# joeyee/Onet

Measured on AMD Instinct MI355X. Metric: training images/sec (twin 256x256 pass), higher is better.
Workload: dtype f32

## Files before the change

### include/onet_hip.h

```cpp
#ifndef ONET_HIP_H
#define ONET_HIP_H

#include <stdint.h>

#ifdef __cplusplus
extern "C" {
#endif

#define ONET_OK 0
#define ONET_EINVAL (-1)
#define ONET_EHIP (-2)

const char* onet_last_error(void);
int onet_abi_version(void);
int onet_device_info(int* cu_count, int* lds_bytes, int* wave_size, char* arch, int arch_len);

int onet_conv3x3_pack_weights(const float* w, float* wp_fwd, float* wp_dgrad,
                              int Cout, int Cin, void* stream);
int onet_convT2x2_pack_weights(const float* w, float* wp_fwd, float* wp_dgrad,
                               int Cin, int Cout, void* stream);
int onet_convT2x2_pack_weights_fused(const float* w, float* wq, int Cin, int Cout, void* stream);
int onet_convT2x2_fwd(const float* x, int64_t x_bs, const float* wq, const float* bias, float* y, int64_t y_bs,
                      int B, int Cin, int Ct, int h, int w, int Ho, int Wo, int pt, int pl, int operand_bf16,
        void* stream);
// ... 4 lines not shown
int onet_convT2x2_dgrad_dbias(const float* dy, int64_t dy_bs, const float* wp_dgrad, float* dx, int64_t dx_bs, float* dbias,
                              void* ws, int64_t ws_bytes, int B, int Cin, int Ct, int h, int w, int Ho, int Wo, int pt, int pl, int operand_bf16,
        void* stream);
int64_t onet_convT2x2_wgrad_ws_bytes(int B, int Cin, int Ct, int h, int w);
int onet_convT2x2_wgrad(const float* x, int64_t x_bs, const float* dy, int64_t dy_bs, float* dw, void* ws,
                        int64_t ws_bytes, int B, int Cin, int Ct, int h, int w, int Ho, int Wo, int pt, int pl, int operand_bf16,
        void* stream);
int onet_convT2x2_dbias(const float* dy, int64_t dy_bs, float* dbias, double* scratch, int accumulate, int B,
                        int C, int h, int w, int Ho, int Wo, int pt, int pl, void* stream);

int onet_conv_fwd(const float* x, int64_t x_bs, const float* wp, float* z, int64_t z_bs,
                  float* bn_part, int B, int Cin, int Cout, int H, int W, int ks, void* stream);
int onet_conv_fwd_nparts(int B, int Cout, int H, int W);

int onet_conv3x3_pack_weights_winograd4(const float* w, float* wq_fwd, float* wq_dgrad,
                                        int Cout, int Cin, void* stream);
int onet_conv3x3_winograd4_fwd(const float* x, int64_t x_bs, const float* wq, float* z, int64_t z_bs,
                               int B, int Cin, int Cout, int H, int W, void* stream);
int onet_conv3x3_winograd4_nparts(int B, int H, int W);
int onet_conv3x3_winograd4_fwd_stats(const float* x, int64_t x_bs, const float* wq, float* z, int64_t z_bs,
                                     float* part, int B, int Cin, int Cout, int H, int W, void* stream);
int onet_conv3x3_winograd4_dgrad_bnreduce(const float* dz, int64_t dz_bs, const float* wq_dgrad, float* da,
                                          int64_t da_bs, const float* z_prev, int64_t z_prev_bs,
                                          const float* save_prev, int group_images, float* part2,
                                          int B, int Cdz, int Cda, int H, int W, void* stream);
int onet_convT2x2_fwd_p(const float* x, int64_t x_bs, const float* wq, const float* bias, void* yP, int64_t yP_bs, const void* y_amax,
                        int nparts, int B, int Cin, int Ct, int h, int w, int Ho, int Wo, int pt, int pl, int operand_bf16, void* stream);
int onet_convT2x2_pack_weights_slots(const float* w, void* wP, void* wdP, void* amax_ws, int Cin, int Ct, int nparts, void* stream);
int onet_convT2x2_fwd_slots(const void* xP, int64_t xP_bs, const void* x_amax, const void* wP, const float* bias, void* yP, int64_t yP_bs,
                            const void* y_amax, int nparts, int B, int Cin, int Ct, int h, int w, void* stream);
int onet_convT2x2_dgrad_slots(const void* dyP, int64_t dyP_bs, const void* dy_amax, const void* wdP, float* dx, int64_t dx_bs, int nparts, int B,
                              int Cin, int Ct, int h, int w, void* stream);
int64_t onet_convT2x2_wgrad_slots_ws_bytes(int B, int Cin, int Ct, int h, int w);
int onet_convT2x2_wgrad_slots(const void* xP, int64_t xP_bs, const void* x_amax, const void* dyP, int64_t dyP_bs, const void* dy_amax, float* dw,
                              float* dbias, void* ws, int64_t ws_bytes, int nparts, int B, int Cin, int Ct, int h, int w, void* stream);
int onet_convT2x2_out_bound(const float* w, const float* bias, int Cin, int Ct, const void* x_amax, void* y_amax, void* stream);

int onet_conv3x3_split_pack_weights(const float* w, void* wq_fwd, void* wq_dgrad, void* amax_ws, int Cout, int Cin, int fwd_f16,
                                    int dgrad_f16, void* stream);
int onet_absmax_slots(const float* x, int64_t n, void* slots, void* stream);
int onet_conv3x3_split_conv_amax(const float* x, int64_t x_bs, const void* x_amax, int scale_always, const void* wq, float* z, int64_t z_bs,
                                 float* part, int B, int Cin, int Cout, int H, int W, void* stream);
int onet_conv3x3_split_wgrad_f16(const float* x, int64_t x_bs, const void* x_amax, const float* save, int n_groups, const float* dz,
                                 int64_t dz_bs, const void* dz_amax, float* dw, void* ws, int64_t ws_bytes, int B, int Cin, int Cout,
                                 int H, int W, int accumulate, void* stream);
int onet_conv3x3_split_fwd(const float* x, int64_t x_bs, const void* wq, int wq_f16, float* z, int64_t z_bs, int B, int Cin, int Cout,
                           int H, int W, void* stream);
int onet_conv3x3_split_nparts(int B, int H, int W);
int onet_split_pack_act(const float* x, int64_t x_bs, void* xs, int64_t xs_bs, int B, int C, int H, int W, int f16, float scale,
                        const void* slots ,
                        void* stream);
int onet_conv3x3_split_dgrad_pre_bnreduce(const void* dzs, int64_t dzs_bs, const void* dz_amax, int scale_always, const void* wq, int wq_f16,
                                          float* da, int64_t da_bs, const void* z_prev, int z_bf16, int64_t z_bs, const float* save, int group_images,
                                          float* rec4, void* da_amax, int B, int Cin, int Cout, int H, int W, void* stream);
int onet_conv3x3_split_fwd_pre(const void* xs, int64_t xs_bs, const void* x_amax, int scale_always, const void* x_amax2, int split_ch,
                               const void* wq, int wq_f16, void* z, int z_bf16 , int64_t z_bs,
                               float* part, int B, int Cin, int Cout, int H, int W,
                               void* stream);
int onet_conv3x3_split_dgrad_pre_slots(const void* dzs, int64_t dzs_bs, const void* dz_amax, int scale_always, const void* wq, int wq_f16,
                                       float* da, int64_t da_bs, void* daP, int64_t daP_bs, int ch0, const void* daP_amax, int B, int Cin,
                                       int Cout, int H, int W, void* stream);
int onet_conv3x3_dgrad_bound(const float* w, int Cout, int Cin, int ci0, const void* dz_amax, void* out_slots, void* stream);
int onet_conv3x3_split_pre_nparts(int B, int H, int W);
int onet_conv3x3_split_wgrad_pre_ok(int B, int Cin, int Cout, int H, int W);
int onet_conv3x3_split_wgrad_pre(const void* xs, int64_t xs_bs, const void* x_amax, const void* x_amax2, int split_ch, const void* dzs,
                                 int64_t dzs_bs, const void* dz_amax, int f16, float* dw, void* ws, int64_t ws_bytes, int B, int Cin,
                                 int Cout, int H, int W, int accumulate, void* stream);
int onet_conv3x3_split_fwd_stats(const float* x, int64_t x_bs, const void* wq, int wq_f16, float* z, int64_t z_bs, float* part, int B,
                                 int Cin, int Cout, int H, int W, void* stream);
int onet_conv3x3_split_wgrad_ok(int B, int Cin, int Cout, int H, int W);
int onet_conv3x3_split_fwd_norm(const float* z_prev, int64_t z_bs, const float* save, int n_groups, const void* wq, int wq_f16,
                                const void* x_amax, float* z, int64_t zo_bs, float* part, int B, int Cin, int Cout, int H, int W,
                                void* stream);
int onet_conv3x3_split_wgrad_norm(const float* z_prev, int64_t z_bs, const float* save, int n_groups, const float* dz, int64_t dz_bs,
                                  float* dw, void* ws, int64_t ws_bytes, int B, int Cin, int Cout, int H, int W, int accumulate,
                                  void* stream);
int64_t onet_conv3x3_split_wgrad_ws_bytes(int B, int Cin, int Cout, int H, int W);
int onet_conv3x3_split_wgrad(const float* x, int64_t x_bs, const float* dz, int64_t dz_bs, float* dw, void* ws, int64_t ws_bytes,
                             int B, int Cin, int Cout, int H, int W, int accumulate, void* stream);

int onet_conv3x3_stem_nparts(int B, int Cin, int Cout, int H, int W);
int onet_conv3x3_stem_fwd_stats(const float* x, int64_t x_bs, const float* w, float* z, int64_t z_bs, float* part, int B, int Cin,
                                int Cout, int H, int W, int twin_B, float twin_bias, void* stream);

int onet_conv3x3_winograd4_wgrad_ok(int B, int Cin, int Cout, int H, int W);
int64_t onet_conv3x3_winograd4_wgrad_ws_bytes(int B, int Cin, int Cout, int H, int W);
int onet_conv3x3_winograd4_wgrad(const float* x, int64_t x_bs, const float* dz, int64_t dz_bs, float* dw, void* ws,
                                 int64_t ws_bytes, int B, int Cin, int Cout, int H, int W, int accumulate, void* stream);

int onet_conv_wgrad(const float* x, int64_t x_bs, const float* dz, int64_t dz_bs, float* dw,
                    void* ws, int64_t ws_bytes, int B, int Cin, int Cout, int H, int W, int ks,
                    int out_layout, int accumulate, void* stream);
int onet_conv3x3_stem_wgrad_bn(const float* x, int64_t x_bs, const float* da, int64_t da_bs, const float* z, int64_t z_bs, const float* save,
                               const float* coef, int group_images, float* dw, void* ws, int64_t ws_bytes, int B, int Cin, int Cout, int H,
                               int W, int accumulate, int twin_B, float twin_bias, void* stream);
int64_t onet_conv_wgrad_ws_bytes(int B, int Cin, int Cout, int H, int W, int ks);

int onet_bn_stats_partial(const float* z, int64_t z_bs, float* part, int nparts,
                          int B, int C, int HW, void* stream);
int onet_bn_finalize(const float* part, int nparts, int64_t count, const float* gamma, const float* beta, float* running_mean,
                     float* running_var, float momentum, float eps, float* save, void* act_amax, int C, void* stream);
int onet_bn_finalize_cm(const float* part, int nparts, int64_t c_stride, const float* gamma, const float* beta, float* running_mean,
                        float* running_var, float momentum, float eps, float* save, void* act_amax, int groups, int C, void* stream);
int onet_bn_eval_coeffs(const float* gamma, const float* beta, const float* running_mean,
                        const float* running_var, float eps, float* save, int C, void* stream);
int onet_bn_relu_apply(const void* z, int z_bf16, int64_t z_bs, float* a, int64_t a_bs, const float* save, void* amax, int group_images,
                       int B, int C, int HW, void* stream);
int onet_bn_relu_apply_pool(const float* z, int64_t z_bs, float* a, int64_t a_bs, float* y, int64_t y_bs, const float* save,
                            void* amax, int B, int C, int H, int W, void* stream);

int onet_bn_relu_bwd_reduce(const float* da, int64_t da_bs, const void* z, int z_bf16, int64_t z_bs, const float* save, float* part2,
                            int nparts, void* da_amax, int group_images, int B, int C, int HW, void* stream);
int onet_bn_bwd_finalize(const float* part2, int nparts, int64_t count, float* dgamma, float* dbeta, float* coef, int accumulate,
                         int groups, int C, const float* save, const void* da_amax, void* dz_amax, void* stream);
int onet_bn_bwd_finalize_cm(const float* part2, int nparts, int64_t c_stride, int64_t count, float* dgamma,
                            float* dbeta, float* coef, int accumulate, int C, void* stream);
int onet_bn_relu_bwd_apply(const float* da, int64_t da_bs, const float* z, int64_t z_bs, const float* save, const float* coef,
                           float* dz, int64_t dz_bs, void* amax, int group_images, int B, int C, int HW, void* stream);
int onet_bn_relu_apply_split(const void* z, int z_bf16, int64_t z_bs, void* xs, int64_t xs_bs, float* a, int64_t a_bs, const float* save,
                             const void* act_amax, int nparts, int group_images, int B, int C, int H, int W, void* stream);
int onet_bn_relu_apply_pool_split(const void* z, int z_bf16, int64_t z_bs, void* xs, int64_t xs_bs, float* a, int64_t a_bs, void* ys, int64_t ys_bs,
                                  float* y, int64_t y_bs, const float* save, const void* act_amax, int nparts, int group_images, int B, int C,
                                  int H, int W, void* stream);
int onet_bn_bwd_bound(const float* save, const float* coef, const void* da_amax, int64_t count, void* dz_amax, int C, void* stream);
int onet_bn_relu_bwd_apply_split(const float* da, int64_t da_bs, const void* z, int z_bf16, int64_t z_bs, const float* save, const float* coef,
                                 void* dzs, int64_t dzs_bs, const void* dz_amax, int nparts, int group_images, int B, int C, int H, int W,
                                 void* stream);
int onet_bn_relu_bwd_apply_split_gl(const float* L, int64_t L_bs, const float* g, const float* z, int64_t z_bs, const float* save,
                                    const float* coef, void* dzs, int64_t dzs_bs, const void* dz_amax, int nparts, int group_images, int B, int C,
                                    int H, int W, void* stream);

int onet_maxpool2_fwd(const float* x, int64_t x_bs, float* y, int64_t y_bs,
                      int B, int C, int H, int W, void* stream);
int onet_maxpool2_bwd(const float* x, int64_t x_bs, const float* dy, int64_t dy_bs, const float* add, int64_t add_bs,
                      const float* add2, int64_t add2_bs, float* dx, int64_t dx_bs, int B, int C, int H, int W, int accumulate,
                      void* stream);
int onet_maxpool2_bwd_bn_bands(int H, int W);
int onet_maxpool2_bwd_add_bnreduce(const float* x, int64_t x_bs, const float* dy, int64_t dy_bs, const float* add, int64_t add_bs,
                                        const float* add2, int64_t add2_bs, float* dx, int64_t dx_bs, const void* z, int z_bf16, int64_t z_bs,
                                        const float* save, int group_images, float* part2, void* dx_amax, int B, int C, int H, int W,
                                        void* stream);

int onet_pixel_shuffle2_bias(const float* sub, const float* bias, float* y, int64_t y_bs,
                             int B, int C, int h, int w, int Ho, int Wo, int pt, int pl, void* stream);
int onet_space_to_depth2(const float* dy, int64_t dy_bs, float* sub, float* dbias, double* scratch,
                         int accumulate, int B, int C, int h, int w, int Ho, int Wo, int pt, int pl,
                         void* stream);
int onet_copy_strided(const float* src, int64_t src_bs, float* dst, int64_t dst_bs,
                      int B, int64_t n, void* stream);

int onet_bilinear2x_fwd(const float* x, int64_t x_bs, float* y, int64_t y_bs, int B, int C,
                        int h, int w, int Ho, int Wo, int pt, int pl, void* stream);
int onet_bilinear2x_bwd(const float* dy, int64_t dy_bs, float* dx, int64_t dx_bs, int B, int C,
                        int h, int w, int Ho, int Wo, int pt, int pl, void* stream);

int onet_complement_clip(const float* x, float* y, float bias, int64_t n, void* stream);

int onet_head_softmax_fwd(const float* Lt, int64_t Lt_bs, const float* Ht, int64_t Ht_bs, const float* Ld, int64_t Ld_bs, const float* Hd,
                          int64_t Hd_bs, float* Vt, float* Vd, float* S, float* sLt, float* sLd, const float* h_save_t, const float* h_save_d,
                          int B, int C, int HW, void* stream);
int onet_head_softmax_bwd(const float* dVt, const float* dVd, const float* dS, const float* gsLt, const float* gsLd, const float* S,
                          const float* Lt, int64_t Lt_bs, const float* Ht, int64_t Ht_bs, const float* Ld, int64_t Ld_bs, const float* Hd,
                          int64_t Hd_bs, float* dLt, float* dHt, float* dLd, float* dHd, const float* h_save_t, const float* h_save_d, int B,
                          int C, int HW, void* stream);

int onet_head_grad_map(const float* dVt, const float* dVd, const float* dS, const float* S, float* g, int B, int HW, void* stream);
int onet_head_bwd_reduce(const float* L, int64_t L_bs, const float* z, int64_t z_bs, const float* g, const float* gsLt, const float* gsLd,
                         const float* save, float* dL, float* part2, int nparts, void* da_amax, int B, int C, int HW, void* stream);

int onet_jsd_fwd(const float* L, int64_t L_bs, const float* Si, int64_t Si_bs,
                 const float* Sp, int64_t Sp_bs, float* sums, double* part, float* jsd,
                 int B, int C, int HW, void* stream);
int onet_jsd_nparts(void);
int onet_jsd_bwd(const float* gscale, const float* sums, const float* Si, int64_t Si_bs,
                 const float* Sp, int64_t Sp_bs, float* gL, float* dSi, float* dSp,
                 int B, int HW, void* stream);
int onet_log1pexp_inplace(float* x, int64_t n, void* stream);
int onet_log1pexp_bwd(const float* x, const float* g, float* out, int64_t n, void* stream);
// ... 27 lines not shown
```

### onet_amd/csrc/bn.hip

```cpp
#include <type_traits>
#include "common.hpp"

using namespace onet;

__global__ __launch_bounds__(256) void bn_stats_partial_kernel(const float* __restrict__ z, int64_t z_bs,
                                                               float* __restrict__ part, int C, int HW,
                                                               int chunks, int chunk_len) {
    __shared__ double red[16];
    const int c = blockIdx.x % C;
    const int p = blockIdx.x / C;
    const int b = p / chunks, ch = p % chunks;
    const float* src = z + (int64_t)b * z_bs + (int64_t)c * HW;
    const int beg = ch * chunk_len;
    const int end = min(beg + chunk_len, HW);
    const bool vec = ((HW & 3) == 0) && ((z_bs & 3) == 0) && ((chunk_len & 3) == 0);
    const double pivot = (double)src[beg];
    double v[2] = {0.0, 0.0};
    if (vec) {
        int i = beg + threadIdx.x * 4;
        for (; i + 3072 < end; i += 4096) {
            float4 q[4];
#pragma unroll
            for (int k = 0; k < 4; ++k) q[k] = *reinterpret_cast<const float4*>(src + i + 1024 * k);
#pragma unroll
            for (int k = 0; k < 4; ++k) {
                const double d0 = q[k].x - pivot, d1 = q[k].y - pivot, d2 = q[k].z - pivot, d3 = q[k].w - pivot;
                v[0] += (d0 + d1) + (d2 + d3);
                v[1] += (d0 * d0 + d1 * d1) + (d2 * d2 + d3 * d3);
            }
        }
        for (; i < end; i += 1024) {
            const float4 q = *reinterpret_cast<const float4*>(src + i);
            const double d0 = q.x - pivot, d1 = q.y - pivot, d2 = q.z - pivot, d3 = q.w - pivot;
            v[0] += (d0 + d1) + (d2 + d3);
            v[1] += (d0 * d0 + d1 * d1) + (d2 * d2 + d3 * d3);
        }
    } else {
        for (int i = beg + threadIdx.x; i < end; i += 256) {
            const double d = src[i] - pivot;
            v[0] += d;
            v[1] += d * d;
        }
    }
    block_sum_256<double, 2>(v, red);
    if (threadIdx.x == 0) {
        const double n = (double)(end - beg);
        const double mean = pivot + v[0] / n;
        double m2 = v[1] - v[0] * v[0] / n;
        if (m2 < 0.0) m2 = 0.0;
        float* o = part + ((int64_t)p * C + c) * 3;
        o[0] = (float)n;
        o[1] = (float)mean;
        o[2] = (float)(m2 + n * (mean - (double)(float)mean) * (mean - (double)(float)mean));
    }
}

__global__ __launch_bounds__(64) void bn_finalize_kernel(const float* __restrict__ part, int nparts,
                                                         const float* __restrict__ gamma,
                                                         const float* __restrict__ beta, float* running_mean,
                                                         float* running_var, float momentum, float eps,
                                                         float* __restrict__ save, int C, unsigned* __restrict__ act_slots = nullptr) {
    const int c = blockIdx.x;
    double n = 0.0, s = 0.0;
    for (int p = threadIdx.x; p < nparts; p += 64) {
        const float* o = part + ((int64_t)p * C + c) * 3;
        n += (double)o[0];
        s += (double)o[0] * (double)o[1];
    }
    n = wave_sum(n);
    s = wave_sum(s);
    const double mean = s / n;
    double m2 = 0.0;
    for (int p = threadIdx.x; p < nparts; p += 64) {
        const float* o = part + ((int64_t)p * C + c) * 3;
        const double d = (double)o[1] - mean;
        m2 += (double)o[2] + (double)o[0] * d * d;
    }
    m2 = wave_sum(m2);
    if (threadIdx.x == 0) {
        const double var = m2 / n;
        const float invstd = (float)(1.0 / sqrt(var + (double)eps));
        const float g = gamma ? gamma[c] : 1.f, bt = beta ? beta[c] : 0.f;
        const float scale = g * invstd;
        save[c] = (float)mean;
// ... 252 lines not shown
        lds[1280 + 5 * t + q] = mid;
    }
    __syncthreads();
    bn_u32x4* dst = reinterpret_cast<bn_u32x4*>(xs);
#pragma unroll
    for (int j = 0; j < 8; ++j) {
        const int part = j >> 2, px = (j & 3) * 256 + t;
        if (part >= np) break;
        const int64_t a = addr(px);
        if (a >= 0) dst[a + (int64_t)part * mid_off] = lds[part * 1280 + px + (px >> 2)];
    }
}

__device__ __forceinline__ void bn_store_slots_block(bn_u32x4* lds, unsigned* __restrict__ xs, int c8, int H, int W, int p_blk, int HW,
                                                     const float (&v)[4][8], float s, int np = 2) {
    if (np == 1) {
        bn_store_slots_block_fn(lds, xs, 0, v, s, [&](int px) -> int64_t {
            const int p = p_blk + px;
            if (p >= HW) return -1;
            int y, x;
            bn_pixel_of(p, W, y, x);
            return (int64_t)(c8 * H + y) * W + x;
        }, 1);
        return;
    }
    const int t = threadIdx.x;
#pragma unroll
    for (int q = 0; q < 4; ++q) {
        bn_u32x4 hi, mid;
#pragma unroll
        for (int k = 0; k < 4; ++k) {
            unsigned h, m;
            split2h_s(v[q][2 * k], v[q][2 * k + 1], s, h, m);
            hi[k] = h;
            mid[k] = m;
        }
        lds[5 * t + q] = hi;
        lds[1280 + 5 * t + q] = mid;
    }
    __syncthreads();
    bn_u32x4* dst = reinterpret_cast<bn_u32x4*>(xs);
#pragma unroll
    for (int j = 0; j < 8; ++j) {
        const int part = j >> 2, px = (j & 3) * 256 + t, p = p_blk + px;
        if (p < HW) {
            int y, x;
            bn_pixel_of(p, W, y, x);
            dst[((int64_t)(c8 * H + y) * 2 + part) * W + x] = lds[part * 1280 + px + (px >> 2)];
        }
    }
}

template <typename ZT = float>
__global__ __launch_bounds__(256) void bn_relu_apply_split_kernel(const ZT* __restrict__ z, int64_t z_bs, unsigned* __restrict__ xs,
                                                                  int64_t xs_bs, float* __restrict__ a, int64_t a_bs,
                                                                  const float* __restrict__ save, int C, int H, int W, int bpp, int np,
                                                                  const unsigned* __restrict__ slots, int gimg) {
    float s_inv;
    const float s_act = np == 1 ? 1.f : amax_scale(amax_read(slots), false, s_inv);
    const int plane = blockIdx.x / bpp, blk = blockIdx.x % bpp;
    const int C8 = C >> 3, b = plane / C8, c8 = plane % C8;
    if (gimg) save += (int64_t)(b / gimg) * 4 * C;
    bn_u32x4* const tr = bn_tr_lds();
    const int HW = H * W, p = (blk * 256 + threadIdx.x) * 4;
    const bool live = p < HW;
    const ZT* src = z + (int64_t)b * z_bs + (int64_t)c8 * 8 * HW + p;
    float v[4][8];
#pragma unroll
    for (int k = 0; k < 8; ++k) {
        const int c = c8 * 8 + k;
        const float mean = save[c], sc = save[2 * C + c], sh = save[3 * C + c];
        const float4 q = live ? bn_ldz4<ZT>(src + (int64_t)k * HW) : make_float4(0.f, 0.f, 0.f, 0.f);
        v[0][k] = fmaxf(fmaf(q.x - mean, sc, sh), 0.f);
        v[1][k] = fmaxf(fmaf(q.y - mean, sc, sh), 0.f);
        v[2][k] = fmaxf(fmaf(q.z - mean, sc, sh), 0.f);
        v[3][k] = fmaxf(fmaf(q.w - mean, sc, sh), 0.f);
    }
    if (a && live) {
        float* d = a + (int64_t)b * a_bs + (int64_t)c8 * 8 * HW + p;
#pragma unroll
        for (int k = 0; k < 8; ++k) *reinterpret_cast<float4*>(d + (int64_t)k * HW) = make_float4(v[0][k], v[1][k], v[2][k], v[3][k]);
    }
    bn_store_slots_block(tr, xs + (int64_t)b * xs_bs, c8, H, W, blk * 1024, HW, v, s_act, np);
}

template <typename ZT = float>
__global__ __launch_bounds__(256) void bn_relu_apply_pool_split_kernel(const ZT* __restrict__ z, int64_t z_bs, unsigned* __restrict__ xs,
                                                                       int64_t xs_bs, float* __restrict__ a, int64_t a_bs,
                                                                       unsigned* __restrict__ ys, int64_t ys_bs, float* __restrict__ yf,
                                                                       int64_t yf_bs, const float* __restrict__ save, int C, int H, int W,
                                                                       int bpp, int np, const unsigned* __restrict__ slots, int gimg) {
    float s_inv;
    const float s_act = np == 1 ? 1.f : amax_scale(amax_read(slots), false, s_inv);
    const int plane = blockIdx.x / bpp, blk = blockIdx.x % bpp;
    const int C8 = C >> 3, b = plane / C8, c8 = plane % C8;
    if (gimg) save += (int64_t)(b / gimg) * 4 * C;
    const int Hp = H >> 1, Wp = W >> 1, W4 = W >> 2, HW = H * W, i = blk * 256 + threadIdx.x;
    const bool live = i < Hp * W4;
    int yo, q;
    bn_pixel_of(live ? i : 0, W4, yo, q);
    const int64_t in_off = (int64_t)c8 * 8 * HW + (int64_t)(2 * yo) * W + 4 * q;
    const ZT* src = z + (int64_t)b * z_bs + in_off;
    float v[8][8], m[2][8];
#pragma unroll
    for (int k = 0; k < 8; ++k) {
        const int c = c8 * 8 + k;
        const float mean = save[c], sc = save[2 * C + c], sh = save[3 * C + c];
        const float4 r0 = bn_ldz4<ZT>(src + (int64_t)k * HW), r1 = bn_ldz4<ZT>(src + (int64_t)k * HW + W);
        v[0][k] = fmaxf(fmaf(r0.x - mean, sc, sh), 0.f);
        v[1][k] = fmaxf(fmaf(r0.y - mean, sc, sh), 0.f);
        v[2][k] = fmaxf(fmaf(r0.z - mean, sc, sh), 0.f);
        v[3][k] = fmaxf(fmaf(r0.w - mean, sc, sh), 0.f);
        v[4][k] = fmaxf(fmaf(r1.x - mean, sc, sh), 0.f);
        v[5][k] = fmaxf(fmaf(r1.y - mean, sc, sh), 0.f);
        v[6][k] = fmaxf(fmaf(r1.z - mean, sc, sh), 0.f);
        v[7][k] = fmaxf(fmaf(r1.w - mean, sc, sh), 0.f);
        m[0][k] = fmaxf(fmaxf(v[0][k], v[1][k]), fmaxf(v[4][k], v[5][k]));
        m[1][k] = fmaxf(fmaxf(v[2][k], v[3][k]), fmaxf(v[6][k], v[7][k]));
    }
    if (a && live) {
        float* d = a + (int64_t)b * a_bs + in_off;
#pragma unroll
        for (int k = 0; k < 8; ++k) {
            *reinterpret_cast<float4*>(d + (int64_t)k * HW) = make_float4(v[0][k], v[1][k], v[2][k], v[3][k]);
            *reinterpret_cast<float4*>(d + (int64_t)k * HW + W) = make_float4(v[4][k], v[5][k], v[6][k], v[7][k]);
        }
    }
    if (xs) {
        bn_u32x4* const tr = bn_tr_lds();
        unsigned* o = xs + (int64_t)b * xs_bs;
        const int npatch = Hp * W4, patch0 = blk * 256;
#pragma unroll
        for (int r = 0; r < 2; ++r) {
            if (r) __syncthreads();
            float vr[4][8];
#pragma unroll
            for (int e = 0; e < 4; ++e)
#pragma unroll
                for (int k = 0; k < 8; ++k) vr[e][k] = live ? v[4 * r + e][k] : 0.f;
            bn_store_slots_block_fn(tr, o, W, vr, s_act, [&](int px) -> int64_t {
                const int pi = patch0 + (px >> 2);
                if (pi >= npatch) return -1;
                int py, pq;
                bn_pixel_of(pi, W4, py, pq);
                return ((int64_t)(c8 * H + 2 * py + r) * np) * W + 4 * pq + (px & 3);
            }, np);
        }
    }
    if (!live) return;
    if (ys) {
        unsigned* o = ys + (int64_t)b * ys_bs;
        bn_store_slots(o, ((int64_t)(c8 * Hp + yo) * np) * Wp + 2 * q, Wp, m[0], s_act, np);
        bn_store_slots(o, ((int64_t)(c8 * Hp + yo) * np) * Wp + 2 * q + 1, Wp, m[1], s_act, np);
    }
    if (yf) {
        float* d = yf + (int64_t)b * yf_bs + (int64_t)c8 * 8 * Hp * Wp + (int64_t)yo * Wp + 2 * q;
#pragma unroll
        for (int k = 0; k < 8; ++k) *reinterpret_cast<float2*>(d + (int64_t)k * Hp * Wp) = make_float2(m[0][k], m[1][k]);
    }
}

constexpr int BN_BWD_OCC16 = 4;
template <typename ZT = float, bool GL = false>
__global__ __launch_bounds__(256, sizeof(ZT) == 2 ? BN_BWD_OCC16 : 3) void bn_relu_bwd_apply_split_kernel(const float* __restrict__ da, int64_t da_bs, const ZT* __restrict__ z,
                                                                      int64_t z_bs, const float* __restrict__ save, const float* __restrict__ coef,
                                                                      unsigned* __restrict__ dzs, int64_t dzs_bs, const unsigned* __restrict__ slots,
// ... 55 lines not shown
__global__ __launch_bounds__(64) void bn_bwd_bound_kernel(const float* __restrict__ save, const float* __restrict__ coef,
                                                          const unsigned* __restrict__ da_slots, float xhat_max, unsigned* __restrict__ dz_slots,
                                                          int C) {
    const float da_max = amax_read(da_slots);
    float bound = 0.f;
    for (int c = blockIdx.x * 64 + threadIdx.x; c < C; c += gridDim.x * 64) {
        const float c1 = coef ? fabsf(coef[c]) + fabsf(coef[C + c]) : 0.f, c2 = coef ? fabsf(coef[2 * C + c]) + fabsf(coef[3 * C + c]) : 0.f;
        bound = fmaxf(bound, fabsf(save[2 * C + c]) * (da_max + c1 + c2 * xhat_max));
    }
#pragma unroll
    for (int o = 32; o > 0; o >>= 1) bound = fmaxf(bound, __shfl_xor(bound, o, 64));
    if (threadIdx.x == 0 && bound == bound) atomicMax(dz_slots + (blockIdx.x & 63) * AMAX_STRIDE, __builtin_bit_cast(unsigned, bound));
}

template <typename ZT = float>
__global__ __launch_bounds__(256) void bn_relu_bwd_reduce_kernel(const float* __restrict__ da, int64_t da_bs,
                                                                 const ZT* __restrict__ z, int64_t z_bs,
                                                                 const float* __restrict__ save,
                                                                 float* __restrict__ part2, int C, int HW,
                                                                 int chunks, int chunk_len, unsigned* __restrict__ amax = nullptr,
                                                                 int gimg = 0) {
    __shared__ double red[8];
    float vmax = 0.f;
    const int c = blockIdx.x % C;
    const int p = blockIdx.x / C;
    const int b = p / chunks, ch = p % chunks;
    if (gimg) save += (int64_t)(b / gimg) * 4 * C;
    const float mean = save[c], invstd = save[C + c], sc = save[2 * C + c], sh = save[3 * C + c];
    const double meand = mean, invd = invstd;
    const ZT* zs = z + (int64_t)b * z_bs + (int64_t)c * HW;
    const float* ds = da + (int64_t)b * da_bs + (int64_t)c * HW;
    const int beg = ch * chunk_len, end = min(beg + chunk_len, HW);
    double v[2] = {0.0, 0.0};
    if (((HW & 3) == 0) && ((z_bs & 3) == 0) && ((da_bs & 3) == 0) && ((chunk_len & 3) == 0)) {
        int i = beg + threadIdx.x * 4;
        for (; i + 3072 < end; i += 4096) {
            float4 q[4], g[4];
#pragma unroll
            for (int k = 0; k < 4; ++k) {
                q[k] = bn_ldz4<ZT>(zs + i + 1024 * k);
                g[k] = *reinterpret_cast<const float4*>(ds + i + 1024 * k);
            }
#pragma unroll
            for (int k = 0; k < 4; ++k) {
                const float zz[4] = {q[k].x, q[k].y, q[k].z, q[k].w}, gg[4] = {g[k].x, g[k].y, g[k].z, g[k].w};
#pragma unroll
                for (int e = 0; e < 4; ++e) {
                    const double dy = fmaf(zz[e] - mean, sc, sh) > 0.f ? (double)gg[e] : 0.0;
                    v[0] += dy;
                    v[1] += dy * (((double)zz[e] - meand) * invd);
                    vmax = fmaxf(vmax, fabsf(gg[e]));
                }
            }
        }
        for (; i < end; i += 1024) {
            const float4 q = bn_ldz4<ZT>(zs + i);
            const float4 g = *reinterpret_cast<const float4*>(ds + i);
            const float zz[4] = {q.x, q.y, q.z, q.w}, gg[4] = {g.x, g.y, g.z, g.w};
#pragma unroll
            for (int k = 0; k < 4; ++k) {
                const double dy = fmaf(zz[k] - mean, sc, sh) > 0.f ? (double)gg[k] : 0.0;
                v[0] += dy;
                v[1] += dy * (((double)zz[k] - meand) * invd);
                vmax = fmaxf(vmax, fabsf(gg[k]));
            }
        }
    } else {
        for (int i = beg + threadIdx.x; i < end; i += 256) {
            const float zi = bn_ldz<ZT>(zs + i);
            const double dy = fmaf(zi - mean, sc, sh) > 0.f ? (double)ds[i] : 0.0;
            v[0] += dy;
            v[1] += dy * (((double)zi - meand) * invd);
            vmax = fmaxf(vmax, fabsf(ds[i]));
        }
    }
    amax_commit(vmax, amax);
    block_sum_256<double, 2>(v, red);
    if (threadIdx.x == 0) {
        float* o = part2 + ((int64_t)p * C + c) * 4;
        o[0] = (float)v[0];
        o[1] = (float)(v[0] - (double)o[0]);
        o[2] = (float)v[1];
        o[3] = (float)(v[1] - (double)o[2]);
    }
}

__global__ __launch_bounds__(256) void head_bwd_reduce_kernel(const float* __restrict__ L, int64_t L_bs, const float* __restrict__ z,
                                                              int64_t z_bs, const float* __restrict__ g, const float* __restrict__ at_t,
                                                              const float* __restrict__ at_d, const float* __restrict__ save,
                                                              float* __restrict__ dL, float* __restrict__ part2, int C, int HW, int chunks,
                                                              int chunk_len, unsigned* __restrict__ amax, int gimg) {
    __shared__ double red[8];
    float vmax = 0.f;
    const int c = blockIdx.x % C;
    const int p = blockIdx.x / C;
    const int b = p / chunks, ch = p % chunks;
    save += (int64_t)(b / gimg) * 4 * C;
    const float mean = save[c], invstd = save[C + c], sc = save[2 * C + c], sh = save[3 * C + c];
    const double meand = mean, invd = invstd;
    const float* zs = z + (int64_t)b * z_bs + (int64_t)c * HW;
    const float* ls = L + (int64_t)b * L_bs + (int64_t)c * HW;
    const float* gs = g + (int64_t)b * HW;
    const float* as = b < gimg ? at_t : at_d;
    if (as) as += (int64_t)(b % gimg) * HW;
    float* os = dL + ((int64_t)b * C + c) * HW;
    const int beg = ch * chunk_len, end = min(beg + chunk_len, HW);
    const float4 zero4 = make_float4(0.f, 0.f, 0.f, 0.f);
    double v[2] = {0.0, 0.0};
    auto four = [&](const float4& q, const float4& l, const float4& gv, const float4& av) -> float4 {
        const float zz[4] = {q.x, q.y, q.z, q.w}, ll[4] = {l.x, l.y, l.z, l.w}, gg[4] = {gv.x, gv.y, gv.z, gv.w}, aa[4] = {av.x, av.y, av.z, av.w};
        float o[4];
#pragma unroll
        for (int e = 0; e < 4; ++e) {
            const float x = fmaf(zz[e] - mean, sc, sh);
            o[e] = fmaf(gg[e], fmaxf(x, 0.f), aa[e]);
            const float da = gg[e] * ll[e];
            const double dy = x > 0.f ? (double)da : 0.0;
            v[0] += dy;
            v[1] += dy * (((double)zz[e] - meand) * invd);
            vmax = fmaxf(vmax, fabsf(da));
        }
        return make_float4(o[0], o[1], o[2], o[3]);
    };
    int i = beg + threadIdx.x * 4;
    for (; i + 3072 < end; i += 4096) {
        float4 q[4], l[4], gv[4], av[4];
#pragma unroll
        for (int k = 0; k < 4; ++k) {
            q[k] = *reinterpret_cast<const float4*>(zs + i + 1024 * k);
            l[k] = *reinterpret_cast<const float4*>(ls + i + 1024 * k);
            gv[k] = *reinterpret_cast<const float4*>(gs + i + 1024 * k);
            av[k] = as ? *reinterpret_cast<const float4*>(as + i + 1024 * k) : zero4;
        }
#pragma unroll
        for (int k = 0; k < 4; ++k) *reinterpret_cast<float4*>(os + i + 1024 * k) = four(q[k], l[k], gv[k], av[k]);
    }
    for (; i < end; i += 1024) {
        const float4 q = *reinterpret_cast<const float4*>(zs + i), l = *reinterpret_cast<const float4*>(ls + i);
        const float4 gv = *reinterpret_cast<const float4*>(gs + i), av = as ? *reinterpret_cast<const float4*>(as + i) : zero4;
        *reinterpret_cast<float4*>(os + i) = four(q, l, gv, av);
    }
    amax_commit(vmax, amax);
    block_sum_256<double, 2>(v, red);
    if (threadIdx.x == 0) {
        float* o = part2 + ((int64_t)p * C + c) * 4;
        o[0] = (float)v[0];
        o[1] = (float)(v[0] - (double)o[0]);
        o[2] = (float)v[1];
        o[3] = (float)(v[1] - (double)o[2]);
    }
}

__global__ __launch_bounds__(256) void bn_bwd_finalize_kernel(const float* __restrict__ part2, int nparts,
                                                             double count, float* dgamma, float* dbeta,
                                                             float* coef, int accumulate, int C, const float* __restrict__ save = nullptr,
                                                             const unsigned* __restrict__ da_slots = nullptr,
                                                             unsigned* __restrict__ dz_slots = nullptr, float xhat_max = 0.f, int groups = 1) {
    __shared__ double wsum[2][4];
    const float da_max = dz_slots ? amax_read(da_slots) : 0.f;
    const int c = blockIdx.x;
    float acc_b = 0.f, acc_g = 0.f;
    if (accumulate && threadIdx.x == 0) {
        acc_b = dbeta ? dbeta[c] : 0.f;
        acc_g = dgamma ? dgamma[c] : 0.f;
    }
    for (int g = 0; g < groups; ++g) {
// ... 148 lines not shown

int onet_bn_stats_partial(const float* z, int64_t z_bs, float* part, int nparts, int B, int C, int HW,
                          void* stream) {
    ONET_REQUIRE(z && part && B > 0 && C > 0 && HW > 0, "bn_stats_partial: bad args");
    int chunks, chunk_len;
    ONET_REQUIRE(split_plan(nparts, B, HW, chunks, chunk_len), "bn_stats_partial: nparts=%d must be a multiple of B=%d", nparts, B);
    hipLaunchKernelGGL(bn_stats_partial_kernel, dim3((unsigned)((int64_t)nparts * C)), dim3(256), 0,
                       as_stream(stream), z, z_bs, part, C, HW, chunks, chunk_len);
    return check_launch("bn_stats_partial_kernel");
}

int onet_bn_finalize(const float* part, int nparts, int64_t count, const float* gamma, const float* beta, float* running_mean,
                         float* running_var, float momentum, float eps, float* save, void* act_amax, int C, void* stream) {
    ONET_REQUIRE(part && save && nparts > 0 && count > 0 && C > 0, "bn_finalize: bad args");
    (void)count;
    hipLaunchKernelGGL(bn_finalize_kernel, dim3(C), dim3(64), 0, as_stream(stream), part, nparts, gamma, beta, running_mean, running_var,
                       momentum, eps, save, C, (unsigned*)act_amax);
    return check_launch("bn_finalize_kernel");
}

int onet_bn_finalize_cm(const float* part, int nparts, int64_t c_stride, const float* gamma, const float* beta, float* running_mean,
                            float* running_var, float momentum, float eps, float* save, void* act_amax, int groups, int C, void* stream) {
    ONET_REQUIRE(part && save && nparts > 0 && C > 0 && groups >= 1 && c_stride >= (int64_t)nparts * groups * 3, "bn_finalize_cm: bad args");
    hipLaunchKernelGGL(bn_finalize_cm_kernel, dim3(C), dim3(256), 0, as_stream(stream), part, nparts, c_stride, gamma, beta, running_mean,
                       running_var, momentum, eps, save, C, (unsigned*)act_amax, groups);
    return check_launch("bn_finalize_cm_kernel");
}

int onet_bn_eval_coeffs(const float* gamma, const float* beta, const float* running_mean,
                        const float* running_var, float eps, float* save, int C, void* stream) {
    ONET_REQUIRE(running_mean && running_var && save && C > 0, "bn_eval_coeffs: bad args");
    hipLaunchKernelGGL(bn_eval_coeffs_kernel, dim3(cdiv(C, 256)), dim3(256), 0, as_stream(stream), gamma, beta,
                       running_mean, running_var, eps, save, C);
    return check_launch("bn_eval_coeffs_kernel");
}

int onet_bn_relu_apply(const void* z, int z_bf16, int64_t z_bs, float* a, int64_t a_bs, const float* save, void* amax, int group_images,
                            int B, int C, int HW, void* stream) {
    ONET_REQUIRE(z && a && save && B > 0 && C > 0 && HW > 0 && group_images >= 0, "bn_relu_apply: bad args");
    const int chunks = cdiv(HW, 4096);
    const int64_t blocks = (int64_t)B * C * chunks;
    ONET_REQUIRE(blocks < (1ll << 31), "bn_relu_apply: grid too large");
    if (z_bf16) {
        ONET_REQUIRE((reinterpret_cast<uintptr_t>(z) & 7) == 0, "bn_relu_apply: 8-byte aligned bf16 rows required");
        hipLaunchKernelGGL(bn_relu_apply_kernel<__bf16>, dim3((unsigned)blocks), dim3(256), 0, as_stream(stream), (const __bf16*)z, z_bs, a, a_bs,
                           save, C, HW, chunks, (unsigned*)amax, group_images);
    } else {
        hipLaunchKernelGGL(bn_relu_apply_kernel<float>, dim3((unsigned)blocks), dim3(256), 0, as_stream(stream), (const float*)z, z_bs, a, a_bs,
                           save, C, HW, chunks, (unsigned*)amax, group_images);
    }
    return check_launch("bn_relu_apply_kernel");
}

int onet_bn_relu_apply_pool(const float* z, int64_t z_bs, float* a, int64_t a_bs, float* y, int64_t y_bs, const float* save,
                                 void* amax, int B, int C, int H, int W, void* stream) {
    ONET_REQUIRE(z && a && y && save && B > 0 && C > 0 && H > 0 && W > 0, "bn_relu_apply_pool: bad args");
    auto al = [](const void* p, uintptr_t m) { return (reinterpret_cast<uintptr_t>(p) & m) == 0; };
    if ((H & 1) || (W & 3) || (z_bs & 3) || (a_bs & 3) || (y_bs & 1) || !al(z, 15) || !al(a, 15) || !al(y, 7)) return 1;
    const int npatch = (H / 2) * (W / 4), bpp = cdiv(npatch, 256);
    const int64_t blocks = (int64_t)B * C * bpp;
    ONET_REQUIRE(blocks < (1ll << 31), "bn_relu_apply_pool: grid too large");
    hipLaunchKernelGGL(bn_relu_apply_pool_kernel, dim3((unsigned)blocks), dim3(256), 0, as_stream(stream), z, z_bs, a, a_bs,
                       y, y_bs, save, C, H, W, bpp, (unsigned*)amax);
    return check_launch("bn_relu_apply_pool_kernel");
}

int onet_bn_relu_bwd_reduce(const float* da, int64_t da_bs, const void* z, int z_bf16, int64_t z_bs, const float* save, float* part2,
                                 int nparts, void* da_amax, int group_images, int B, int C, int HW, void* stream) {
    ONET_REQUIRE(da && z && save && part2 && B > 0 && C > 0 && HW > 0 && group_images >= 0, "bn_relu_bwd_reduce: bad args");
    int chunks, chunk_len;
    ONET_REQUIRE(split_plan(nparts, B, HW, chunks, chunk_len), "bn_relu_bwd_reduce: nparts=%d must be a multiple of B=%d", nparts, B);
    const dim3 grid((unsigned)((int64_t)nparts * C));
    if (z_bf16) {
        ONET_REQUIRE((reinterpret_cast<uintptr_t>(z) & 7) == 0, "bn_relu_bwd_reduce: 8-byte aligned bf16 rows required");
        hipLaunchKernelGGL(bn_relu_bwd_reduce_kernel<__bf16>, grid, dim3(256), 0, as_stream(stream), da, da_bs, (const __bf16*)z, z_bs, save,
                           part2, C, HW, chunks, chunk_len, (unsigned*)da_amax, group_images);
    } else {
        hipLaunchKernelGGL(bn_relu_bwd_reduce_kernel<float>, grid, dim3(256), 0, as_stream(stream), da, da_bs, (const float*)z, z_bs, save,
                           part2, C, HW, chunks, chunk_len, (unsigned*)da_amax, group_images);
    }
    return check_launch("bn_relu_bwd_reduce_kernel");
}

int onet_bn_bwd_bound(const float* save, const float* coef, const void* da_amax, int64_t count, void* dz_amax, int C, void* stream) {
    ONET_REQUIRE(save && da_amax && dz_amax && count > 0 && C > 0, "bn_bwd_bound: bad args");
    hipLaunchKernelGGL(bn_bwd_bound_kernel, dim3(cdiv(C, 64)), dim3(64), 0, as_stream(stream), save, coef, (const unsigned*)da_amax,
                       sqrtf((float)(count > 1 ? count - 1 : 1)), (unsigned*)dz_amax, C);
    return check_launch("bn_bwd_bound_kernel");
}

int onet_bn_relu_apply_split(const void* z, int z_bf16, int64_t z_bs, void* xs, int64_t xs_bs, float* a, int64_t a_bs, const float* save,
                             const void* act_amax, int nparts, int group_images, int B, int C, int H, int W, void* stream) {
    ONET_REQUIRE(nparts == 1 || nparts == 2, "bn_relu_apply_split: nparts must be 2 (fp16 hi | mid) or 1 (plain bf16)");
    ONET_REQUIRE(z && xs && save && B > 0 && C > 0 && (C % 8) == 0 && H > 0 && W > 0 && (W % 4) == 0, "bn_relu_apply_split: bad args (C %% 8 == 0, W %% 4 == 0)");
    ONET_REQUIRE((reinterpret_cast<uintptr_t>(xs) & 15) == 0 && (xs_bs & 3) == 0 && (reinterpret_cast<uintptr_t>(z) & 15) == 0 && (z_bs & 3) == 0 &&
                 (reinterpret_cast<uintptr_t>(a) & 15) == 0 && (a_bs & 3) == 0, "bn_relu_apply_split: 16-byte aligned rows and slots required");
    const int bpp = cdiv((int64_t)H * W, 1024);
    const int64_t blocks = (int64_t)B * (C / 8) * bpp;
    ONET_REQUIRE(blocks < (1ll << 31) && (int64_t)H * W < (1 << 24), "bn_relu_apply_split: grid too large");
    if (z_bf16)
        hipLaunchKernelGGL(bn_relu_apply_split_kernel<__bf16>, dim3((unsigned)blocks), dim3(256), bn_tr_bytes(nparts), as_stream(stream), (const __bf16*)z, z_bs,
                           (unsigned*)xs, xs_bs, a, a_bs, save, C, H, W, bpp, nparts, (const unsigned*)act_amax, group_images);
    else
        hipLaunchKernelGGL(bn_relu_apply_split_kernel<float>, dim3((unsigned)blocks), dim3(256), bn_tr_bytes(nparts), as_stream(stream), (const float*)z, z_bs,
                           (unsigned*)xs, xs_bs, a, a_bs, save, C, H, W, bpp, nparts, (const unsigned*)act_amax, group_images);
    return check_launch("bn_relu_apply_split_kernel");
}

int onet_bn_relu_apply_pool_split(const void* z, int z_bf16, int64_t z_bs, void* xs, int64_t xs_bs, float* a, int64_t a_bs, void* ys, int64_t ys_bs,
                                  float* y, int64_t y_bs, const float* save, const void* act_amax, int nparts, int group_images, int B, int C,
                                  int H, int W, void* stream) {
    ONET_REQUIRE(nparts == 1 || nparts == 2, "bn_relu_apply_pool_split: nparts must be 2 (fp16 hi | mid) or 1 (plain bf16)");
    ONET_REQUIRE(z && (xs || a) && (ys || y) && save && B > 0 && C > 0 && (C % 8) == 0 && H > 0 && W > 0, "bn_relu_apply_pool_split: bad args");
    auto al = [](const void* p, uintptr_t m) { return (reinterpret_cast<uintptr_t>(p) & m) == 0; };
    if ((H & 1) || (W & 3) || (z_bs & 3) || (a_bs & 3) || (xs_bs & 3) || (ys_bs & 3) || (y_bs & 1) || !al(z, 15) || !al(a, 15) || !al(xs, 15) ||
        !al(ys, 15) || !al(y, 7))
        return 1;
    const int bpp = cdiv((int64_t)(H / 2) * (W / 4), 256);
    const int64_t blocks = (int64_t)B * (C / 8) * bpp;
    ONET_REQUIRE(blocks < (1ll << 31) && (int64_t)H * W < (1 << 24), "bn_relu_apply_pool_split: grid too large");
    if (z_bf16)
        hipLaunchKernelGGL(bn_relu_apply_pool_split_kernel<__bf16>, dim3((unsigned)blocks), dim3(256), bn_tr_bytes(nparts), as_stream(stream), (const __bf16*)z, z_bs,
                           (unsigned*)xs, xs_bs, a, a_bs, (unsigned*)ys, ys_bs, y, y_bs, save, C, H, W, bpp, nparts, (const unsigned*)act_amax,
                           group_images);
    else
        hipLaunchKernelGGL(bn_relu_apply_pool_split_kernel<float>, dim3((unsigned)blocks), dim3(256), bn_tr_bytes(nparts), as_stream(stream), (const float*)z, z_bs,
                           (unsigned*)xs, xs_bs, a, a_bs, (unsigned*)ys, ys_bs, y, y_bs, save, C, H, W, bpp, nparts, (const unsigned*)act_amax,
                           group_images);
    return check_launch("bn_relu_apply_pool_split_kernel");
}

int onet_bn_relu_bwd_apply_split(const float* da, int64_t da_bs, const void* z, int z_bf16, int64_t z_bs, const float* save, const float* coef,
                                 void* dzs, int64_t dzs_bs, const void* dz_amax, int nparts, int group_images, int B, int C, int H, int W,
                                 void* stream) {
    ONET_REQUIRE(nparts == 1 || nparts == 2, "bn_relu_bwd_apply_split: nparts must be 2 (fp16 hi | mid) or 1 (plain bf16)");
    ONET_REQUIRE(da && z && save && dzs && (dz_amax || nparts == 1) && B > 0 && C > 0 && (C % 8) == 0 && H > 0 && W > 0 && (W % 4) == 0,
                 "bn_relu_bwd_apply_split: bad args");
    ONET_REQUIRE((reinterpret_cast<uintptr_t>(dzs) & 15) == 0 && (dzs_bs & 3) == 0 && (reinterpret_cast<uintptr_t>(z) & 15) == 0 && (z_bs & 3) == 0 &&
                 (reinterpret_cast<uintptr_t>(da) & 15) == 0 && (da_bs & 3) == 0, "bn_relu_bwd_apply_split: 16-byte aligned rows and slots required");
    const int bpp = cdiv((int64_t)H * W, 1024);
    const int64_t blocks = (int64_t)B * (C / 8) * bpp;
    ONET_REQUIRE(blocks < (1ll << 31) && (int64_t)H * W < (1 << 24), "bn_relu_bwd_apply_split: grid too large");
    if (z_bf16)
        hipLaunchKernelGGL(bn_relu_bwd_apply_split_kernel<__bf16>, dim3((unsigned)blocks), dim3(256), bn_tr_bytes(nparts), as_stream(stream), da, da_bs,
                           (const __bf16*)z, z_bs, save, coef, (unsigned*)dzs, dzs_bs, (const unsigned*)dz_amax, C, H, W, bpp, nparts, group_images);
    else
        hipLaunchKernelGGL(bn_relu_bwd_apply_split_kernel<float>, dim3((unsigned)blocks), dim3(256), bn_tr_bytes(nparts), as_stream(stream), da, da_bs,
                           (const float*)z, z_bs, save, coef, (unsigned*)dzs, dzs_bs, (const unsigned*)dz_amax, C, H, W, bpp, nparts, group_images);
    return check_launch("bn_relu_bwd_apply_split_kernel");
}

int onet_head_bwd_reduce(const float* L, int64_t L_bs, const float* z, int64_t z_bs, const float* g, const float* gsLt, const float* gsLd,
                         const float* save, float* dL, float* part2, int nparts, void* da_amax, int B, int C, int HW, void* stream) {
    ONET_REQUIRE(L && z && g && save && dL && part2 && B > 0 && (B % 2) == 0 && C > 0 && HW > 0, "head_bwd_reduce: bad args (B = images of the twin batch)");
    auto al = [](const void* q) { return (reinterpret_cast<uintptr_t>(q) & 15) == 0; };
    ONET_REQUIRE((HW & 3) == 0 && (L_bs & 3) == 0 && (z_bs & 3) == 0 && al(L) && al(z) && al(g) && al(gsLt) && al(gsLd) && al(dL),
                 "head_bwd_reduce: HW %% 4 == 0 and 16-byte aligned rows required");
    int chunks, chunk_len;
    ONET_REQUIRE(split_plan(nparts, B, HW, chunks, chunk_len), "head_bwd_reduce: nparts=%d must be a multiple of B=%d", nparts, B);
    ONET_REQUIRE((int64_t)nparts * C < (1ll << 31), "head_bwd_reduce: grid too large");
    hipLaunchKernelGGL(head_bwd_reduce_kernel, dim3((unsigned)((int64_t)nparts * C)), dim3(256), 0, as_stream(stream), L, L_bs, z, z_bs, g, gsLt,
                       gsLd, save, dL, part2, C, HW, chunks, chunk_len, (unsigned*)da_amax, B / 2);
    return check_launch("head_bwd_reduce_kernel");
}

int onet_bn_relu_bwd_apply_split_gl(const float* L, int64_t L_bs, const float* g, const float* z, int64_t z_bs, const float* save,
// ... 45 lines not shown
```

### onet_amd/csrc/common.hpp

```cpp
#pragma once
#include <hip/hip_runtime.h>
#include <stdint.h>
#include <atomic>
#include <stdio.h>
#include "../../include/onet_hip.h"

namespace onet {

void set_error(const char* fmt, ...);
int check_launch(const char* what);

#define ONET_REQUIRE(cond, ...)                    \
    do {                                           \
        if (!(cond)) {                             \
            onet::set_error(__VA_ARGS__);          \
            return ONET_EINVAL;                    \
        }                                          \
    } while (0)

static inline hipStream_t as_stream(void* s) { return reinterpret_cast<hipStream_t>(s); }

static inline int cdiv(int64_t a, int64_t b) { return (int)((a + b - 1) / b); }

struct PerDeviceOnce {
    std::atomic<uint64_t> seen{0};
    bool first() {
        int d = 0;
        (void)hipGetDevice(&d);
        const uint64_t bit = 1ull << (d & 63);
        return !(seen.fetch_or(bit, std::memory_order_relaxed) & bit);
    }
};

inline int device_cu_count() {
    static std::atomic<int> cached[64];
    int d = 0;
    (void)hipGetDevice(&d);
    int n = cached[d & 63].load(std::memory_order_relaxed);
    if (n <= 0) {
        if (hipDeviceGetAttribute(&n, hipDeviceAttributeMultiprocessorCount, d) != hipSuccess || n <= 0) n = 256;
        cached[d & 63].store(n, std::memory_order_relaxed);
    }
    return n;
}

template <typename T>
__device__ __forceinline__ T wave_sum(T v) {
#pragma unroll
    for (int o = 32; o > 0; o >>= 1) v += __shfl_xor(v, o, 64);
    return v;
}

template <typename T, int NV>
__device__ __forceinline__ void block_sum_256(T (&v)[NV], T* smem ) {
    const int lane = threadIdx.x & 63, wid = threadIdx.x >> 6;
#pragma unroll
    for (int i = 0; i < NV; ++i) v[i] = wave_sum(v[i]);
    if (lane == 0) {
#pragma unroll
        for (int i = 0; i < NV; ++i) smem[wid * NV + i] = v[i];
    }
    __syncthreads();
    if (threadIdx.x == 0) {
#pragma unroll
        for (int i = 0; i < NV; ++i) v[i] = smem[i] + smem[NV + i] + smem[2 * NV + i] + smem[3 * NV + i];
    }
}

__device__ __forceinline__ void split2h_s(float a, float b, float s, unsigned& hi, unsigned& mid) {
    unsigned h, m;
    asm("v_fma_mixlo_f16 %0, %1, %3, 0 op_sel_hi:[0,0,0]\n\tv_fma_mixhi_f16 %0, %2, %3, 0 op_sel_hi:[0,0,0]"
        : "=&v"(h) : "v"(a), "v"(b), "v"(s));
    asm("v_fma_mixlo_f16 %0, %1, %3, -%4 op_sel:[0,0,0] op_sel_hi:[0,0,1]\n\tv_fma_mixhi_f16 %0, %2, %3, -%4 op_sel:[0,0,1] op_sel_hi:[0,0,1]"
        : "=&v"(m) : "v"(a), "v"(b), "v"(s), "v"(h));
    hi = h;
    mid = m;
}

constexpr int AMAX_SLOTS = 64, AMAX_STRIDE = 32;
__device__ __forceinline__ float amax_read(const unsigned* slots) {
    if (!slots) return 0.f;
    unsigned v = slots[(threadIdx.x & (AMAX_SLOTS - 1)) * AMAX_STRIDE];
#pragma unroll
    for (int o = 32; o > 0; o >>= 1) v = max(v, (unsigned)__shfl_xor((int)v, o, 64));
    return __builtin_bit_cast(float, __builtin_amdgcn_readfirstlane(v));
}
__device__ __forceinline__ float amax_scale(float amax, bool always, float& inv) {
    const unsigned bits = __builtin_bit_cast(unsigned, amax);
    const int e = (int)((bits >> 23) & 255u) - 127;
    int k = 0;
    if (bits != 0u && e < 128) k = (always || e >= 15) ? 13 - e : 0;
    k = max(-100, min(100, k));
    inv = __builtin_bit_cast(float, (unsigned)(127 - k) << 23);
    return __builtin_bit_cast(float, (unsigned)(127 + k) << 23);
}

int launch_wgrad_reduce(const float* slab, float* dw, int splitK, int taps, int Cout, int Cin, int out_layout, int accumulate,
                        hipStream_t st);

int convt_gemm_fwd(const float* x, int64_t x_bs, const float* wq, const float* bias, float* y, int64_t y_bs, void* y16, int64_t y16_bs,
                   int B, int Cin, int Ct, int h, int w, int Ho, int Wo, int pt, int pl, int prec, hipStream_t st, int y16_split = 0,
                   const void* out_slots = nullptr);
int convt_out_bound(const float* w, const float* bias, int Cin, int Ct, const void* x_slots, void* out_slots, hipStream_t st);
int64_t convt_gemm_dbias_ws_bytes(int B, int Ct, int h, int w);
int convt_gemm_dgrad(const float* dy, int64_t dy_bs, const float* wd, float* dx, int64_t dx_bs, float* dbias, float* dbias_ws, int B,
                     int Cin, int Ct, int h, int w, int Ho, int Wo, int pt, int pl, int prec, hipStream_t st);
int64_t convt_gemm_wgrad_ws_bytes(int B, int Cin, int Ct, int h, int w);
int convt_gemm_wgrad(const float* x, int64_t x_bs, const float* dy, int64_t dy_bs, float* dw, void* ws, int64_t ws_bytes, int B,
                     int Cin, int Ct, int h, int w, int Ho, int Wo, int pt, int pl, int prec, hipStream_t st);

}
```

### onet_amd/csrc/conv_mfma.hip

```cpp
#include <algorithm>
#include <cstdlib>
#include "common.hpp"

using namespace onet;

typedef float f32x16 __attribute__((ext_vector_type(16)));

__global__ void pack3x3_kernel(const float* __restrict__ w, float* __restrict__ wf,
                               float* __restrict__ wd, int Cout, int Cin) {
    int64_t n = (int64_t)Cout * Cin * 9;
    for (int64_t i = blockIdx.x * (int64_t)blockDim.x + threadIdx.x; i < n;
         i += (int64_t)gridDim.x * blockDim.x) {
        int t = (int)(i % 9);
        int64_t r = i / 9;
        int ci = (int)(r % Cin), co = (int)(r / Cin);
        float v = w[i];
        if (wf) wf[((int64_t)ci * 9 + t) * Cout + co] = v;
        if (wd) wd[((int64_t)co * 9 + (8 - t)) * Cin + ci] = v;
    }
}

__global__ void packT2x2_kernel(const float* __restrict__ w, float* __restrict__ wf,
                                float* __restrict__ wd, float* __restrict__ wq, int Cin, int Cout) {
    int64_t n = (int64_t)Cin * Cout * 4;
// ... 245 lines not shown
                            if (vec2) {
                                *reinterpret_cast<float2*>(o) = make_float2(v0, v1);
                                *reinterpret_cast<float2*>(o + a.Wo) = make_float2(v2, v3);
                            } else {
                                o[0] = v0; o[1] = v1; o[a.Wo] = v2; o[a.Wo + 1] = v3;
                            }
                        }
                    }
                }
            }
        }
        return;
    }
#pragma unroll
    for (int m = 0; m < MT; ++m) {
#pragma unroll
        for (int n = 0; n < NT; ++n) {
            const int yo = y0 + (wn * NT + n) * RPT + py;
            if (yo < a.H && xo < a.W) {
#pragma unroll
                for (int r = 0; r < 16; ++r) {
                    const int co = co0 + (wm * MT + m) * 32 + (r & 3) + 8 * (r >> 2) + 4 * kh;
                    if (co < a.Cout) zb[(int64_t)co * HW + (int64_t)yo * a.W + xo] = acc[m][n][r];
                }
            }
        }
    }
}

template <int KS, int MT, int NT, int WM, int WN, int TW, int MODE = 0>
static int launch_fwd(ConvArgs a, hipStream_t st) {
    using C = ConvCfg<KS, MT, NT, WM, WN, TW>;
    a.tilesX = cdiv(a.W, TW);
    a.tilesY = cdiv(a.H, C::ROWS);
    a.coTiles = cdiv(a.Cout, C::CO_T);
    const int64_t blocks = (int64_t)a.B * a.tilesX * a.tilesY * a.coTiles;
    ONET_REQUIRE(blocks > 0 && blocks < (1ll << 31), "conv_fwd: grid %lld out of range", (long long)blocks);
    auto kern = conv_fwd_kernel<KS, MT, NT, WM, WN, TW, MODE>;
    static PerDeviceOnce attr_once;
    if (attr_once.first()) {
        (void)hipFuncSetAttribute(reinterpret_cast<const void*>(kern), hipFuncAttributeMaxDynamicSharedMemorySize,
                                  C::LDS_BYTES);
    }
    hipLaunchKernelGGL(kern, dim3((unsigned)blocks), dim3(256), C::LDS_BYTES, st, a);
    return check_launch("conv_fwd_kernel");
}

static int conv_cfg_override() {
    static int v = -1;
    if (v < 0) {
        const char* e = getenv("ONET_CONV_CFG");
        v = (e && e[0]) ? e[0] : 0;
    }
    return v;
}

template <int KS>
static int dispatch_fwd(const ConvArgs& a, hipStream_t st) {
    const bool wide = a.W > 16;
    if (!wide) return launch_fwd<KS, 2, 2, 1, 4, 16>(a, st);
    switch (conv_cfg_override()) {
        case 'P': return launch_fwd<KS, 2, 4, 1, 4, 32>(a, st);
        case 'C': return launch_fwd<KS, 2, 4, 2, 2, 32>(a, st);
        case 'D': return launch_fwd<KS, 2, 2, 1, 4, 32>(a, st);
        case 'E': return launch_fwd<KS, 2, 2, 2, 2, 32>(a, st);
        default: break;
    }
    return launch_fwd<KS, 2, 2, 1, 4, 32>(a, st);
}

struct WgArgs {
    const float* x;
    int64_t x_bs;
    const float* dz;
    int64_t dz_bs;
    float* slab;
    int B, Cin, Cout, H, W, ciTiles, coTiles, splitK, stripsY, stripsX;
    int s2d_Ct = 0, Ho = 0, Wo = 0, pt = 0, pl = 0;
    const float* bn_z = nullptr;
    int64_t bn_z_bs = 0;
    const float* bn_save = nullptr;
    const float* bn_coef = nullptr;
    int bn_gimg = 0;
    int twin_B = 0;
    float twin_bias = 0.f;
};

template <int KS, int PW>
struct WgCfg {
    static constexpr int TAPS = KS * KS, PAD = KS / 2;
    static constexpr int PR = 64 / PW;
    static constexpr int XR = PR + 2 * PAD, XC = PW + 2 * PAD;
    static constexpr int DZ_STRIDE = PR * PW + 1;
    static constexpr int X_STRIDE = (XR * XC) | 1;
    static constexpr int LDS_BYTES = 64 * (DZ_STRIDE + X_STRIDE) * 4;
};

template <int KS, int PW, bool S2D = false>
__global__ __launch_bounds__(256 * KS, KS == 3 ? 3 : 2) void conv_wgrad_kernel(WgArgs a) {
    using C = WgCfg<KS, PW>;
    constexpr int TAPS = C::TAPS, PAD = C::PAD, PR = C::PR, XR = C::XR, XC = C::XC;
    constexpr int DZ_STRIDE = C::DZ_STRIDE, X_STRIDE = C::X_STRIDE;
    constexpr int TG = KS;
    constexpr int NTAP = TAPS / TG;
    constexpr int NTHR = 256 * TG;
    constexpr int DZ_CSTEP = NTHR / 64;
    constexpr int NDZ = (64 + DZ_CSTEP - 1) / DZ_CSTEP;
    constexpr int ROWS_PER_K = NTHR / PW;
    constexpr int CH_PER_K = ROWS_PER_K / XR;
    constexpr int NXM = (64 + CH_PER_K - 1) / CH_PER_K;
    constexpr int NXH = (KS == 3) ? (64 * XR * 2 + NTHR - 1) / NTHR : 0;

    extern __shared__ __attribute__((aligned(16))) float smem[];
    float* dz_lds = smem;
    float* x_lds = smem + 64 * DZ_STRIDE;

    int bid;
    {
        const int n = gridDim.x, q = n >> 3, r = n & 7, xcd = blockIdx.x & 7, j = blockIdx.x >> 3;
        bid = (xcd < r ? xcd * (q + 1) : r * (q + 1) + (xcd - r) * q) + j;
    }
    const int tiles = a.ciTiles * a.coTiles;
    const int ks = bid / tiles;
    const int tile = bid % tiles;
    const int ciT = tile % a.ciTiles;
    const int coT = tile / a.ciTiles;
    const int co0 = coT * 64, ci0 = ciT * 64;

    const int tid = threadIdx.x, lane = tid & 63, wid = tid >> 6;
    const int tg = wid >> 2, wm = (wid >> 1) & 1, wn = wid & 1;
    const int l31 = lane & 31, kh = lane >> 5;
    const int HW = a.H * a.W;

    f32x16 acc[NTAP];
#pragma unroll
    for (int t = 0; t < NTAP; ++t)
#pragma unroll
        for (int r = 0; r < 16; ++r) acc[t][r] = 0.f;

    const float* a_ptr = dz_lds + (wm * 32 + l31) * DZ_STRIDE + kh;
    const float* b_ptr = x_lds + (wn * 32 + l31) * X_STRIDE + kh + tg * XC;

    const int dz_c = tid >> 6, dz_p = tid & 63, dz_r = dz_p / PW, dz_col = dz_p % PW;
    const int xm_col = tid % PW, xm_rowid = tid / PW, xm_cp = xm_rowid / XR, xm_r = xm_rowid % XR;
    const bool xm_thread = xm_rowid < CH_PER_K * XR;
    const unsigned dz_kstep = (unsigned)(DZ_CSTEP * HW * 4), xm_kstep = (unsigned)(CH_PER_K * HW * 4);

    float dzv[NDZ], xmv[NXM], xhv[NXH > 0 ? NXH : 1];
    const int nunits = a.B * a.stripsY * a.stripsX;

    auto issue = [&](int u) {
        const bool live = u < nunits;
        const int uu = live ? u : 0;
        const int sx = uu % a.stripsX;
        const int sy = (uu / a.stripsX) % a.stripsY;
        const int b = uu / (a.stripsX * a.stripsY);
        const int y0 = sy * PR, x0 = sx * PW;
        const int HWo = a.Ho * a.Wo;
        const __amdgpu_buffer_rsrc_t dr = make_rsrc(a.dz + (int64_t)b * a.dz_bs, S2D ? (int64_t)a.s2d_Ct * HWo * 4 : (int64_t)a.Cout * HW * 4);
        const __amdgpu_buffer_rsrc_t xr = make_rsrc(a.x + (int64_t)b * a.x_bs, (int64_t)a.Cin * HW * 4);
        {
            const int yy = y0 + dz_r, xx = x0 + dz_col;
            const bool ok = live && yy < a.H && xx < a.W;
            unsigned base, kstep;
            if constexpr (S2D) {
                const int q = co0 / a.s2d_Ct, cc = co0 % a.s2d_Ct + dz_c;
// ... 35 lines not shown
                if (xm_cp + CH_PER_K * k < 64)
                    x_lds[(xm_cp + CH_PER_K * k) * X_STRIDE + xm_r * XC + xm_col + PAD] = xmv[k];
        }
#pragma unroll
        for (int j = 0; j < NXH; ++j) {
            const int e = tid + NTHR * j;
            const int c = e / (2 * XR), q = e % (2 * XR);
            if (e < 64 * XR * 2) x_lds[c * X_STRIDE + (q >> 1) * XC + ((q & 1) ? XC - 1 : 0)] = xhv[j];
        }
    };

    issue(ks);
    for (int u = ks; u < nunits; u += a.splitK) {
        commit();
        __syncthreads();
        issue(u + a.splitK);
        __builtin_amdgcn_sched_barrier(0);
#pragma unroll
        for (int r = 0; r < PR; ++r) {
#pragma unroll
            for (int j = 0; j < PW / 2; ++j) {
                const float av = a_ptr[r * PW + 2 * j];
#pragma unroll
                for (int t = 0; t < NTAP; ++t) {
                    const float bv = b_ptr[r * XC + 2 * j + t];
                    acc[t] = __builtin_amdgcn_mfma_f32_32x32x2f32(av, bv, acc[t], 0, 0, 0);
                }
            }
        }
        __syncthreads();
    }
    float* sl = a.slab + (int64_t)ks * TAPS * a.Cout * a.Cin;
    const int ci = ci0 + wn * 32 + l31;
    if (ci < a.Cin) {
#pragma unroll
        for (int t = 0; t < NTAP; ++t) {
#pragma unroll
            for (int r = 0; r < 16; ++r) {
                const int co = co0 + wm * 32 + (r & 3) + 8 * (r >> 2) + 4 * kh;
                if (co < a.Cout) sl[((int64_t)(tg * NTAP + t) * a.Cout + co) * a.Cin + ci] = acc[t][r];
            }
        }
    }
}

__global__ __launch_bounds__(256) void wgrad_reduce_kernel(const float* __restrict__ slab, float* __restrict__ dw,
                                                           int splitK, int taps, int Cout, int Cin, int out_layout,
                                                           int accumulate) {
    __shared__ float red[256];
    const int64_t n = (int64_t)Cout * Cin;
    const int t = blockIdx.y;
    const int64_t i = (int64_t)blockIdx.x * 64 + (threadIdx.x & 63);
    const int g = threadIdx.x >> 6;
    float s = 0.f;
    if (i < n)
        for (int k = g; k < splitK; k += 4) s += slab[((int64_t)k * taps + t) * n + i];
    red[threadIdx.x] = s;
    __syncthreads();
    if (g == 0 && i < n) {
        s = (red[threadIdx.x] + red[threadIdx.x + 64]) + (red[threadIdx.x + 128] + red[threadIdx.x + 192]);
        const int ci = (int)(i % Cin), co = (int)(i / Cin);
        int64_t o;
        if (out_layout == 0) {
            o = i * taps + t;
        } else {
            const int Ct = Cout / 4, q = co / Ct, cot = co % Ct;
            o = ((int64_t)ci * Ct + cot) * 4 + q;
        }
        dw[o] = accumulate ? dw[o] + s : s;
    }
}

namespace onet {
int launch_wgrad_reduce(const float* slab, float* dw, int splitK, int taps, int Cout, int Cin, int out_layout, int accumulate,
                        hipStream_t st) {
    const int64_t n = (int64_t)Cout * Cin;
    hipLaunchKernelGGL(wgrad_reduce_kernel, dim3((unsigned)cdiv(n, 64), (unsigned)taps), dim3(256), 0, st, slab, dw, splitK,
                       taps, Cout, Cin, out_layout, accumulate);
    return check_launch("wgrad_reduce_kernel");
}
}

constexpr int STEM_ROWS = 32;
template <int CIN, int COG, bool BN = false>
__global__ __launch_bounds__(256) void conv3x3_stem_wgrad_kernel(WgArgs a) {
    constexpr int NV = COG * CIN * 9;
    __shared__ float red[4][NV];
    const int cogs = (a.Cout + COG - 1) / COG;
    const int bandsY = (a.H + STEM_ROWS - 1) / STEM_ROWS;
    const int cg = blockIdx.x % cogs, bb = blockIdx.x / cogs;
    const int b = bb / bandsY, yb = (bb % bandsY) * STEM_ROWS;
    const int tid = threadIdx.x, lane = tid & 63, wid = tid >> 6;
    const int HW = a.H * a.W, W = a.W, H = a.H;
    const bool comp = a.twin_B > 0 && b >= a.twin_B;
    const float* xb = a.x + (int64_t)(comp ? b - a.twin_B : b) * a.x_bs;
    const float* dzb = a.dz + (int64_t)b * a.dz_bs + (int64_t)cg * COG * HW;
    const float* zb = BN ? a.bn_z + (int64_t)b * a.bn_z_bs + (int64_t)cg * COG * HW : nullptr;
    const int y0 = yb + wid * (STEM_ROWS / 4), y1 = min(y0 + STEM_ROWS / 4, H);
    const bool vec = (W & 3) == 0 && (a.dz_bs & 3) == 0 && (reinterpret_cast<uintptr_t>(a.dz) & 15) == 0 &&
                     (!BN || ((a.bn_z_bs & 3) == 0 && (reinterpret_cast<uintptr_t>(a.bn_z) & 15) == 0));
    float bmean[COG], binv[COG], bsc[COG], bsh[COG];
    double bc1[COG], bc2[COG];
    if (BN) {
        const int grp = a.bn_gimg ? b / a.bn_gimg : 0;
        const float* sv = a.bn_save + (int64_t)grp * 4 * a.Cout;
        const float* cf = a.bn_coef ? a.bn_coef + (int64_t)grp * 4 * a.Cout : nullptr;
#pragma unroll
        for (int g = 0; g < COG; ++g) {
            const int c = min(cg * COG + g, a.Cout - 1);
            bmean[g] = sv[c];
            binv[g] = sv[a.Cout + c];
            bsc[g] = sv[2 * a.Cout + c];
            bsh[g] = sv[3 * a.Cout + c];
            bc1[g] = cf ? (double)cf[c] + (double)cf[a.Cout + c] : 0.0;
            bc2[g] = cf ? (double)cf[2 * a.Cout + c] + (double)cf[3 * a.Cout + c] : 0.0;
        }
    }
    float acc[COG][CIN][9];
#pragma unroll
    for (int g = 0; g < COG; ++g)
#pragma unroll
        for (int c = 0; c < CIN; ++c)
#pragma unroll
            for (int t = 0; t < 9; ++t) acc[g][c][t] = 0.f;
    auto in_row = [&](int c, int yy, int x0, float (&r)[6]) __attribute__((always_inline)) {
        const bool rowok = yy >= 0 && yy < H;
        const float* p = xb + (int64_t)c * HW + (int64_t)yy * W;
#pragma unroll
        for (int k = 0; k < 6; ++k) {
            const int xx = x0 - 1 + k;
            const bool ok = rowok && xx >= 0 && xx < W;
            float v = ok ? p[xx] : 0.f;
            if (comp && ok) v = fminf(fmaxf(1.f - v + a.twin_bias, 0.f), 1.f);
            r[k] = v;
        }
    };
    for (int x0 = lane * 4; x0 < W && y0 < y1; x0 += 256) {
        float win[CIN][3][6];
#pragma unroll
        for (int c = 0; c < CIN; ++c) {
            in_row(c, y0 - 1, x0, win[c][1]);
            in_row(c, y0, x0, win[c][2]);
        }
        for (int y = y0; y < y1; ++y) {
#pragma unroll
            for (int c = 0; c < CIN; ++c) {
#pragma unroll
                for (int k = 0; k < 6; ++k) {
                    win[c][0][k] = win[c][1][k];
                    win[c][1][k] = win[c][2][k];
                }
                in_row(c, y + 1, x0, win[c][2]);
            }
#pragma unroll
            for (int g = 0; g < COG; ++g) {
                float gz[4] = {0.f, 0.f, 0.f, 0.f}, zz[4] = {0.f, 0.f, 0.f, 0.f};
                if (cg * COG + g < a.Cout) {
                    const int64_t o = (int64_t)g * HW + (int64_t)y * W + x0;
                    if (vec) {
                        const float4 q = *reinterpret_cast<const float4*>(dzb + o);
                        gz[0] = q.x; gz[1] = q.y; gz[2] = q.z; gz[3] = q.w;
                        if (BN) {
                            const float4 r = *reinterpret_cast<const float4*>(zb + o);
                            zz[0] = r.x; zz[1] = r.y; zz[2] = r.z; zz[3] = r.w;
                        }
                    } else {
#pragma unroll
                        for (int p = 0; p < 4; ++p)
                            if (x0 + p < W) {
                                gz[p] = dzb[o + p];
                                if (BN) zz[p] = zb[o + p];
                            }
                    }
                    if (BN) {
#pragma unroll
                        for (int p = 0; p < 4; ++p) {
                            const double dy = fmaf(zz[p] - bmean[g], bsc[g], bsh[g]) > 0.f ? (double)gz[p] : 0.0;
                            const float v = (float)((double)bsc[g] * (dy - bc1[g] - (((double)zz[p] - (double)bmean[g]) * (double)binv[g]) * bc2[g]));
                            gz[p] = (vec || x0 + p < W) ? v : 0.f;
                        }
                    }
                }
#pragma unroll
                for (int p = 0; p < 4; ++p)
#pragma unroll
                    for (int c = 0; c < CIN; ++c)
#pragma unroll
                        for (int t = 0; t < 9; ++t) acc[g][c][t] = fmaf(gz[p], win[c][t / 3][p + t % 3], acc[g][c][t]);
            }
        }
    }
#pragma unroll
    for (int g = 0; g < COG; ++g)
#pragma unroll
        for (int c = 0; c < CIN; ++c)
#pragma unroll
            for (int t = 0; t < 9; ++t) {
                const float s = wave_sum(acc[g][c][t]);
                if (lane == 0) red[wid][(g * CIN + c) * 9 + t] = s;
            }
    __syncthreads();
    float* sl = a.slab + (int64_t)bb * 9 * a.Cout * CIN;
    for (int i = tid; i < NV; i += 256) {
        const int g = i / (CIN * 9), c = (i / 9) % CIN, t = i % 9;
        const int co = cg * COG + g;
        if (co < a.Cout)
            sl[((int64_t)t * a.Cout + co) * CIN + c] = (red[0][i] + red[1][i]) + (red[2][i] + red[3][i]);
    }
}

template <int KS, int PW, bool S2D = false>
static void launch_wgrad(const WgArgs& a, int64_t blocks, hipStream_t st) {
    using C = WgCfg<KS, PW>;
    auto kern = conv_wgrad_kernel<KS, PW, S2D>;
    static PerDeviceOnce attr_once;
    if (attr_once.first()) {
        (void)hipFuncSetAttribute(reinterpret_cast<const void*>(kern), hipFuncAttributeMaxDynamicSharedMemorySize,
                                  C::LDS_BYTES);
    }
    hipLaunchKernelGGL(kern, dim3((unsigned)blocks), dim3(256 * KS), C::LDS_BYTES, st, a);
}

static void wgrad_plan(int B, int Cin, int Cout, int H, int W, int ks, int& pw, int& splitK,
                       int& stripsX, int& stripsY) {
    pw = (W > 16) ? 32 : 16;
    const int pr = 64 / pw;
    stripsX = cdiv(W, pw);
    stripsY = cdiv(H, pr);
    const int64_t nunits = (int64_t)B * stripsX * stripsY;
    const int64_t tiles = (int64_t)cdiv(Cout, 64) * cdiv(Cin, 64);
    int64_t s = (1024 + tiles - 1) / tiles;
    const int64_t per = (int64_t)ks * ks * Cout * Cin * 4;
    const int64_t cap = (192ll << 20) / (per > 0 ? per : 1);
    if (s > cap) s = cap;
    if (s > nunits) s = nunits;
    if (s < 1) s = 1;
    splitK = (int)s;
}

extern "C" {

int onet_conv3x3_pack_weights(const float* w, float* wp_fwd, float* wp_dgrad, int Cout, int Cin,
                              void* stream) {
    ONET_REQUIRE(w && Cout > 0 && Cin > 0, "pack3x3: bad args");
    const int64_t n = (int64_t)Cout * Cin * 9;
    hipLaunchKernelGGL(pack3x3_kernel, dim3((unsigned)std::min<int64_t>(cdiv(n, 256), 4096)), dim3(256), 0,
                       as_stream(stream), w, wp_fwd, wp_dgrad, Cout, Cin);
    return check_launch("pack3x3_kernel");
}

int onet_convT2x2_pack_weights(const float* w, float* wp_fwd, float* wp_dgrad, int Cin, int Cout,
                               void* stream) {
    ONET_REQUIRE(w && Cout > 0 && Cin > 0, "packT2x2: bad args");
    const int64_t n = (int64_t)Cout * Cin * 4;
    hipLaunchKernelGGL(packT2x2_kernel, dim3((unsigned)std::min<int64_t>(cdiv(n, 256), 4096)), dim3(256), 0,
                       as_stream(stream), w, wp_fwd, wp_dgrad, (float*)nullptr, Cin, Cout);
// ... 51 lines not shown
    ONET_REQUIRE(B > 0 && Cin > 0 && Ct > 0 && h > 0 && w > 0, "convT2x2_dgrad: bad shape");
    ONET_REQUIRE(Ct % CI_T == 0, "convT2x2_dgrad: Ct must be a multiple of %d (use onet_space_to_depth2 + onet_conv_fwd)", CI_T);
    ONET_REQUIRE(pt >= 0 && pl >= 0 && pt + 2 * h <= Ho && pl + 2 * w <= Wo, "convT2x2_dgrad: window outside plane");
    ONET_REQUIRE(dy_bs >= (int64_t)Ct * Ho * Wo && dx_bs >= (int64_t)Cin * h * w, "convT2x2_dgrad: batch stride too small");
    if (convt_gemm_enabled()) {
        const int rc = convt_gemm_dgrad(dy, dy_bs, wp_dgrad, dx, dx_bs, nullptr, nullptr, B, Cin, Ct, h, w, Ho, Wo, pt, pl, operand_bf16, as_stream(stream));
        if (rc <= 0) return rc;
    }
    ConvArgs a{dy, dy_bs, wp_dgrad, dx, dx_bs, nullptr, B, 4 * Ct, Cin, h, w, 0, 0, 0, nullptr, Ho, Wo, pt, pl};
    return (w > 16) ? launch_fwd<1, 2, 2, 1, 4, 32, 2>(a, as_stream(stream))
                    : launch_fwd<1, 2, 2, 1, 4, 16, 2>(a, as_stream(stream));
}

int64_t onet_convT2x2_dgrad_dbias_ws_bytes(int B, int Ct, int h, int w) { return convt_gemm_dbias_ws_bytes(B, Ct, h, w); }

int onet_convT2x2_dgrad_dbias(const float* dy, int64_t dy_bs, const float* wp_dgrad, float* dx, int64_t dx_bs, float* dbias, void* ws,
                              int64_t ws_bytes, int B, int Cin, int Ct, int h, int w, int Ho, int Wo, int pt, int pl, int operand_bf16, void* stream) {
    ONET_REQUIRE(dy && wp_dgrad && dx && dbias && ws, "convT2x2_dgrad_dbias: null pointer");
    ONET_REQUIRE(B > 0 && Cin > 0 && Ct > 0 && h > 0 && w > 0, "convT2x2_dgrad_dbias: bad shape");
    ONET_REQUIRE(dy_bs >= (int64_t)Ct * Ho * Wo && dx_bs >= (int64_t)Cin * h * w, "convT2x2_dgrad_dbias: batch stride too small");
    if (!convt_gemm_enabled() || ws_bytes < convt_gemm_dbias_ws_bytes(B, Ct, h, w)) return 1;
    return convt_gemm_dgrad(dy, dy_bs, wp_dgrad, dx, dx_bs, dbias, (float*)ws, B, Cin, Ct, h, w, Ho, Wo, pt, pl, operand_bf16, as_stream(stream));
}

int onet_conv_fwd_nparts(int B, int Cout, int H, int W) {
    (void)B; (void)Cout; (void)H; (void)W;
    return 0;
}

int onet_conv_fwd(const float* x, int64_t x_bs, const float* wp, float* z, int64_t z_bs, float* bn_part,
                  int B, int Cin, int Cout, int H, int W, int ks, void* stream) {
    ONET_REQUIRE(x && wp && z, "conv_fwd: null pointer");
    ONET_REQUIRE(B > 0 && Cin > 0 && Cout > 0 && H > 0 && W > 0, "conv_fwd: bad shape B=%d Cin=%d Cout=%d H=%d W=%d",
                 B, Cin, Cout, H, W);
    ONET_REQUIRE(ks == 1 || ks == 3, "conv_fwd: ks must be 1 or 3 (got %d)", ks);
    ONET_REQUIRE(bn_part == nullptr, "conv_fwd: fused BN partials not available in this build");
    ONET_REQUIRE(x_bs >= (int64_t)Cin * H * W && z_bs >= (int64_t)Cout * H * W, "conv_fwd: batch stride too small");
    ConvArgs a{x, x_bs, wp, z, z_bs, bn_part, B, Cin, Cout, H, W, 0, 0, 0};
    return ks == 3 ? dispatch_fwd<3>(a, as_stream(stream)) : dispatch_fwd<1>(a, as_stream(stream));
}

static inline bool use_stem_wgrad(int Cin, int ks) { return ks == 3 && Cin <= 4; }
static inline int stem_blocks(int B, int H) { return B * ((H + STEM_ROWS - 1) / STEM_ROWS); }

int64_t onet_conv_wgrad_ws_bytes(int B, int Cin, int Cout, int H, int W, int ks) {
    if (use_stem_wgrad(Cin, ks)) return (int64_t)stem_blocks(B, H) * 9 * Cout * Cin * 4;
    int pw, splitK, sx, sy;
    wgrad_plan(B, Cin, Cout, H, W, ks, pw, splitK, sx, sy);
    return (int64_t)splitK * ks * ks * Cout * Cin * 4;
}

int onet_conv3x3_stem_wgrad_bn(const float* x, int64_t x_bs, const float* da, int64_t da_bs, const float* z, int64_t z_bs, const float* save,
                               const float* coef, int group_images, float* dw, void* ws, int64_t ws_bytes, int B, int Cin, int Cout, int H,
                               int W, int accumulate, int twin_B, float twin_bias, void* stream) {
    ONET_REQUIRE(x && da && z && save && dw && ws, "conv3x3_stem_wgrad_bn: null pointer");
    ONET_REQUIRE(B > 0 && Cin > 0 && Cin <= 4 && Cout > 0 && H > 0 && W > 0 && group_images >= 0 && (group_images == 0 || B % group_images == 0),
                 "conv3x3_stem_wgrad_bn: bad shape (Cin <= 4)");
    WgArgs a{x, x_bs, da, da_bs, (float*)ws, B, Cin, Cout, H, W, 1, cdiv(Cout, 64), 1, 1, 1};
    a.bn_z = z;
    a.bn_z_bs = z_bs;
    a.bn_save = save;
    a.bn_coef = coef;
    a.bn_gimg = group_images;
    ONET_REQUIRE(twin_B == 0 || 2 * twin_B == B, "conv3x3_stem_wgrad_bn: a twin batch holds twin_B = B / 2 images in memory");
    a.twin_B = twin_B;
    a.twin_bias = twin_bias;
    const int nb = stem_blocks(B, H);
    const int64_t need = (int64_t)nb * 9 * Cout * Cin * 4;
    ONET_REQUIRE(ws_bytes >= need, "conv3x3_stem_wgrad_bn: workspace %lld < %lld bytes", (long long)ws_bytes, (long long)need);
    hipStream_t st = as_stream(stream);
    switch (Cin) {
        case 1: hipLaunchKernelGGL((conv3x3_stem_wgrad_kernel<1, 4, true>), dim3(nb * cdiv(Cout, 4)), dim3(256), 0, st, a); break;
        case 2: hipLaunchKernelGGL((conv3x3_stem_wgrad_kernel<2, 2, true>), dim3(nb * cdiv(Cout, 2)), dim3(256), 0, st, a); break;
        case 3: hipLaunchKernelGGL((conv3x3_stem_wgrad_kernel<3, 2, true>), dim3(nb * cdiv(Cout, 2)), dim3(256), 0, st, a); break;
        default: hipLaunchKernelGGL((conv3x3_stem_wgrad_kernel<4, 1, true>), dim3(nb * cdiv(Cout, 1)), dim3(256), 0, st, a); break;
    }
    int rc = check_launch("conv3x3_stem_wgrad_kernel");
    if (rc) return rc;
    const int64_t n = (int64_t)Cout * Cin;
    hipLaunchKernelGGL(wgrad_reduce_kernel, dim3((unsigned)cdiv(n, 64), 9u), dim3(256), 0, st, (const float*)ws, dw, nb, 9, Cout, Cin, 0, accumulate);
    return check_launch("wgrad_reduce_kernel");
}

int onet_conv_wgrad(const float* x, int64_t x_bs, const float* dz, int64_t dz_bs, float* dw, void* ws,
                    int64_t ws_bytes, int B, int Cin, int Cout, int H, int W, int ks, int out_layout,
                    int accumulate, void* stream) {
    ONET_REQUIRE(x && dz && dw && ws, "conv_wgrad: null pointer");
    ONET_REQUIRE(B > 0 && Cin > 0 && Cout > 0 && H > 0 && W > 0, "conv_wgrad: bad shape");
    ONET_REQUIRE(ks == 1 || ks == 3, "conv_wgrad: ks must be 1 or 3 (got %d)", ks);
    ONET_REQUIRE(out_layout == 0 || (out_layout == 1 && ks == 1 && Cout % 4 == 0), "conv_wgrad: bad out_layout");
    WgArgs a{x, x_bs, dz, dz_bs, (float*)ws, B, Cin, Cout, H, W, cdiv(Cin, 64), cdiv(Cout, 64), 1, 1, 1};
    if (use_stem_wgrad(Cin, ks) && out_layout == 0) {
        const int nb = stem_blocks(B, H);
        const int64_t need = (int64_t)nb * 9 * Cout * Cin * 4;
        ONET_REQUIRE(ws_bytes >= need, "conv_wgrad(stem): workspace %lld < %lld bytes", (long long)ws_bytes, (long long)need);
        hipStream_t st = as_stream(stream);
        switch (Cin) {
            case 1: hipLaunchKernelGGL((conv3x3_stem_wgrad_kernel<1, 4>), dim3(nb * cdiv(Cout, 4)), dim3(256), 0, st, a); break;
            case 2: hipLaunchKernelGGL((conv3x3_stem_wgrad_kernel<2, 2>), dim3(nb * cdiv(Cout, 2)), dim3(256), 0, st, a); break;
            case 3: hipLaunchKernelGGL((conv3x3_stem_wgrad_kernel<3, 2>), dim3(nb * cdiv(Cout, 2)), dim3(256), 0, st, a); break;
            default: hipLaunchKernelGGL((conv3x3_stem_wgrad_kernel<4, 1>), dim3(nb * cdiv(Cout, 1)), dim3(256), 0, st, a); break;
        }
        int rc = check_launch("conv3x3_stem_wgrad_kernel");
        if (rc) return rc;
        const int64_t n = (int64_t)Cout * Cin;
        hipLaunchKernelGGL(wgrad_reduce_kernel, dim3((unsigned)cdiv(n, 64), 9u), dim3(256), 0, st,
                           (const float*)ws, dw, nb, 9, Cout, Cin, 0, accumulate);
        return check_launch("wgrad_reduce_kernel");
    }
    int pw;
    wgrad_plan(B, Cin, Cout, H, W, ks, pw, a.splitK, a.stripsX, a.stripsY);
    const int64_t need = (int64_t)a.splitK * ks * ks * Cout * Cin * 4;
    ONET_REQUIRE(ws_bytes >= need, "conv_wgrad: workspace %lld < %lld bytes", (long long)ws_bytes, (long long)need);
    const int64_t blocks = (int64_t)a.splitK * a.ciTiles * a.coTiles;
    hipStream_t st = as_stream(stream);
    if (ks == 3) {
        if (pw == 32) launch_wgrad<3, 32>(a, blocks, st); else launch_wgrad<3, 16>(a, blocks, st);
    } else {
        if (pw == 32) launch_wgrad<1, 32>(a, blocks, st); else launch_wgrad<1, 16>(a, blocks, st);
    }
    int rc = check_launch("conv_wgrad_kernel");
    if (rc) return rc;
    const int64_t n = (int64_t)Cout * Cin;
    hipLaunchKernelGGL(wgrad_reduce_kernel, dim3((unsigned)cdiv(n, 64), (unsigned)(ks * ks)), dim3(256), 0, st,
                       (const float*)ws, dw, a.splitK, ks * ks, Cout, Cin, out_layout, accumulate);
    return check_launch("wgrad_reduce_kernel");
}

int onet_convT2x2_wgrad(const float* x, int64_t x_bs, const float* dy, int64_t dy_bs, float* dw, void* ws,
                        int64_t ws_bytes, int B, int Cin, int Ct, int h, int w, int Ho, int Wo, int pt, int pl, int operand_bf16,
                        void* stream) {
    ONET_REQUIRE(x && dy && dw && ws, "convT2x2_wgrad: null pointer");
    ONET_REQUIRE(B > 0 && Cin > 0 && Ct > 0 && h > 0 && w > 0, "convT2x2_wgrad: bad shape");
    ONET_REQUIRE(Ct % 64 == 0, "convT2x2_wgrad: Ct must be a multiple of 64 (use onet_space_to_depth2 + onet_conv_wgrad)");
    ONET_REQUIRE(pt >= 0 && pl >= 0 && pt + 2 * h <= Ho && pl + 2 * w <= Wo, "convT2x2_wgrad: window outside plane");
    ONET_REQUIRE(dy_bs >= (int64_t)Ct * Ho * Wo && x_bs >= (int64_t)Cin * h * w, "convT2x2_wgrad: batch stride too small");
    if (convt_gemm_enabled()) {
        const int rc = convt_gemm_wgrad(x, x_bs, dy, dy_bs, dw, ws, ws_bytes, B, Cin, Ct, h, w, Ho, Wo, pt, pl, operand_bf16, as_stream(stream));
        if (rc <= 0) return rc;
    }
    const int Cout = 4 * Ct;
    WgArgs a{x, x_bs, dy, dy_bs, (float*)ws, B, Cin, Cout, h, w, cdiv(Cin, 64), cdiv(Cout, 64), 1, 1, 1, Ct, Ho, Wo, pt, pl};
    int pw;
    wgrad_plan(B, Cin, Cout, h, w, 1, pw, a.splitK, a.stripsX, a.stripsY);
    const int64_t need = (int64_t)a.splitK * Cout * Cin * 4;
    ONET_REQUIRE(ws_bytes >= need, "convT2x2_wgrad: workspace %lld < %lld bytes", (long long)ws_bytes, (long long)need);
    const int64_t blocks = (int64_t)a.splitK * a.ciTiles * a.coTiles;
    hipStream_t st = as_stream(stream);
    if (pw == 32) launch_wgrad<1, 32, true>(a, blocks, st); else launch_wgrad<1, 16, true>(a, blocks, st);
    int rc = check_launch("conv_wgrad_kernel");
    if (rc) return rc;
    const int64_t n = (int64_t)Cout * Cin;
    hipLaunchKernelGGL(wgrad_reduce_kernel, dim3((unsigned)cdiv(n, 64), 1u), dim3(256), 0, st, (const float*)ws, dw,
                       a.splitK, 1, Cout, Cin, 1, 0);
    return check_launch("wgrad_reduce_kernel");
}

}
```

### onet_amd/csrc/stem.hip

```cpp
#include <algorithm>
#include "common.hpp"

using namespace onet;

namespace {

struct StemArgs {
    const float* x;
    int64_t x_bs;
    const float* w;
    float* z;
    int64_t z_bs;
    float* part;
    int B, Cout, H, W, tilesX, tilesY;
    int twin_B;
    float twin_bias;
};

constexpr int ST_TH = 16, ST_TW = 64, ST_LR = ST_TH + 2, ST_LC = ST_TW + 4;
constexpr int ST_MAXC = 128;

#define ONET_ST_DPP_ADD(v, ctrl, rmask) \
    v += __builtin_bit_cast(float, __builtin_amdgcn_update_dpp(0, __builtin_bit_cast(int, v), ctrl, rmask, 0xf, false))
__device__ __forceinline__ float wave_sum_hi(float v) {
    ONET_ST_DPP_ADD(v, 0x128, 0xf);
    ONET_ST_DPP_ADD(v, 0x124, 0xf);
    ONET_ST_DPP_ADD(v, 0x122, 0xf);
    ONET_ST_DPP_ADD(v, 0x121, 0xf);
    ONET_ST_DPP_ADD(v, 0x142, 0xa);
    ONET_ST_DPP_ADD(v, 0x143, 0xc);
    return v;
}
#undef ONET_ST_DPP_ADD

template <int CIN>
__global__ __launch_bounds__(256) void stem_conv_stats_kernel(StemArgs a) {
    __shared__ float tile[CIN][ST_LR][ST_LC];
    __shared__ float sc[4][ST_MAXC][2];
    int bid = blockIdx.x;
    const int tx = bid % a.tilesX;
    bid /= a.tilesX;
    const int ty = bid % a.tilesY;
    const int b = bid / a.tilesY;
    const int y0 = ty * ST_TH, x0 = tx * ST_TW;
    const int tid = threadIdx.x, lane = tid & 63, wid = tid >> 6;
    const int HW = a.H * a.W;
    const bool comp = a.twin_B > 0 && b >= a.twin_B;
    const float* xb = a.x + (int64_t)(comp ? b - a.twin_B : b) * a.x_bs;

    for (int i = tid; i < CIN * ST_LR * 66; i += 256) {
        const int ci = i / (ST_LR * 66), r = (i / 66) % ST_LR, c = i % 66;
        const int yy = y0 - 1 + r, xx = x0 - 1 + c;
        const bool ok = yy >= 0 && yy < a.H && xx >= 0 && xx < a.W;
        float v = ok ? xb[(int64_t)ci * HW + (int64_t)yy * a.W + xx] : 0.f;
        if (comp && ok) v = fminf(fmaxf(1.f - v + a.twin_bias, 0.f), 1.f);
        tile[ci][r][c] = v;
    }
    __syncthreads();

    const int r = tid >> 4, q = tid & 15;
    float win[CIN][3][6];
#pragma unroll
    for (int ci = 0; ci < CIN; ++ci)
#pragma unroll
        for (int dy = 0; dy < 3; ++dy)
#pragma unroll
            for (int dx = 0; dx < 6; ++dx) win[ci][dy][dx] = tile[ci][r + dy][4 * q + dx];

    float* zb = a.z + (int64_t)b * a.z_bs + (int64_t)(y0 + r) * a.W + x0 + 4 * q;
    for (int co = 0; co < a.Cout; ++co) {
        const float* wp = a.w + (int64_t)co * CIN * 9;
        float acc[4] = {0.f, 0.f, 0.f, 0.f};
#pragma unroll
        for (int ci = 0; ci < CIN; ++ci)
#pragma unroll
            for (int dy = 0; dy < 3; ++dy)
#pragma unroll
                for (int dx = 0; dx < 3; ++dx) {
                    const float wv = wp[(ci * 3 + dy) * 3 + dx];
#pragma unroll
                    for (int j = 0; j < 4; ++j) acc[j] = fmaf(wv, win[ci][dy][dx + j], acc[j]);
                }
        *reinterpret_cast<float4*>(zb + (int64_t)co * HW) = make_float4(acc[0], acc[1], acc[2], acc[3]);
        if (a.part) {
            const float pv = __builtin_bit_cast(float, __builtin_amdgcn_readfirstlane(__builtin_bit_cast(int, acc[0])));
            float s1 = 0.f, s2 = 0.f;
#pragma unroll
            for (int j = 0; j < 4; ++j) {
                const float d = acc[j] - pv;
                s1 += d;
                s2 = fmaf(d, d, s2);
            }
            s1 = wave_sum_hi(s1);
            s2 = wave_sum_hi(s2);
            if (lane == 63) {
                sc[wid][co][0] = fmaf(s1, 1.f / 256.f, pv);
                sc[wid][co][1] = fmaxf(fmaf(-s1 * (1.f / 256.f), s1, s2), 0.f);
            }
        }
    }
    if (a.part) {
        __syncthreads();
        if (tid < a.Cout) {
            float mw[4], qw[4];
#pragma unroll
            for (int w = 0; w < 4; ++w) {
                mw[w] = sc[w][tid][0];
                qw[w] = sc[w][tid][1];
            }
            const float mean = 0.25f * ((mw[0] + mw[1]) + (mw[2] + mw[3]));
            float m2 = (qw[0] + qw[1]) + (qw[2] + qw[3]);
#pragma unroll
            for (int w = 0; w < 4; ++w) m2 = fmaf(256.f * (mw[w] - mean), mw[w] - mean, m2);
            const int64_t nblk = (int64_t)a.B * a.tilesY * a.tilesX;
            const int64_t blk = ((int64_t)b * a.tilesY + ty) * a.tilesX + tx;
            float* sp = a.part + ((int64_t)tid * nblk + blk) * 3;
            sp[0] = 1024.f;
            sp[1] = mean;
            sp[2] = m2;
        }
    }
}

int stem_nparts(int B, int Cin, int Cout, int H, int W) {
    if (B <= 0 || Cin < 1 || Cin > 4 || Cout < 1 || Cout > ST_MAXC || H <= 0 || W <= 0 || (H % ST_TH) || (W % ST_TW)) return 0;
    const int64_t n = (int64_t)B * (H / ST_TH) * (W / ST_TW);
    return n < (1 << 30) ? (int)n : 0;
}

}

extern "C" {

int onet_conv3x3_stem_nparts(int B, int Cin, int Cout, int H, int W) { return stem_nparts(B, Cin, Cout, H, W); }

int onet_conv3x3_stem_fwd_stats(const float* x, int64_t x_bs, const float* w, float* z, int64_t z_bs, float* part, int B, int Cin,
                                int Cout, int H, int W, int twin_B, float twin_bias, void* stream) {
    ONET_REQUIRE(x && w && z, "conv3x3_stem_fwd_stats: null pointer");
    ONET_REQUIRE(stem_nparts(B, Cin, Cout, H, W) > 0,
                 "conv3x3_stem_fwd_stats: needs 1 <= Cin <= 4, Cout <= %d and a map made of full 16 x 64 tiles (onet_conv3x3_stem_nparts() == 0 elsewhere)",
                 ST_MAXC);
    ONET_REQUIRE(x_bs >= (int64_t)Cin * H * W && z_bs >= (int64_t)Cout * H * W, "conv3x3_stem_fwd_stats: batch stride too small");
    ONET_REQUIRE((z_bs & 3) == 0 && (reinterpret_cast<uintptr_t>(z) & 15) == 0, "conv3x3_stem_fwd_stats: 16-byte aligned output rows required");
    ONET_REQUIRE(twin_B == 0 || 2 * twin_B == B, "conv3x3_stem_fwd_stats: a twin batch holds twin_B = B / 2 images in memory");
    StemArgs a{x, x_bs, w, z, z_bs, part, B, Cout, H, W, W / ST_TW, H / ST_TH, twin_B, twin_bias};
    const int64_t blocks = (int64_t)B * a.tilesX * a.tilesY;
    const dim3 g((unsigned)blocks), t(256);
    switch (Cin) {
        case 1: hipLaunchKernelGGL(stem_conv_stats_kernel<1>, g, t, 0, as_stream(stream), a); break;
        case 2: hipLaunchKernelGGL(stem_conv_stats_kernel<2>, g, t, 0, as_stream(stream), a); break;
        case 3: hipLaunchKernelGGL(stem_conv_stats_kernel<3>, g, t, 0, as_stream(stream), a); break;
        default: hipLaunchKernelGGL(stem_conv_stats_kernel<4>, g, t, 0, as_stream(stream), a); break;
    }
    return check_launch("stem_conv_stats_kernel");
}

}
```

### onet_amd/functional.py

```python
from __future__ import annotations

import torch

from . import ops


def _carries_settings(cls):
    fwd, bwd = cls.forward, cls.backward

    def forward(ctx, *args, **kw):
        ctx._onet_settings = ops.active_settings()
        return fwd(ctx, *args, **kw)

    def backward(ctx, *grads):
        if torch.is_grad_enabled():
            raise RuntimeError("onet_amd: double differentiation (create_graph=True) is not supported: the HIP backward kernels "
                               "build no graph of their own")
        with ops.using(getattr(ctx, "_onet_settings", None)):
            return bwd(ctx, *grads)

    forward.__doc__, backward.__doc__ = fwd.__doc__, bwd.__doc__
    cls.forward, cls.backward = staticmethod(forward), staticmethod(backward)
    return cls

# ... 27 lines not shown
        defer = defer and training and out is None and want_pool is None
        norm = None
        if link_in is not None and link_in.get("deferred"):
            norm = (link_in["z"], link_in["save"], link_in.get("slots"))
        x_amax = aux.get("x_amax") if (aux is not None and norm is None) else None
        if norm is not None:
            z, cm = ops.conv3x3_fwd_bn_partials(None, packed, norm=norm)
        else:
            z, cm = ops.conv3x3_fwd_bn_partials(x, packed, amax=x_amax) if training else (ops.conv3x3_auto(x, packed, 0, amax=x_amax), None)
        dst = None if out is None else out[0]
        G = groups if (training and groups > 1) else 1
        C = z.shape[1]
        save_all = torch.empty((G, 4, C), dtype=torch.float32, device=z.device)
        Bz, _, Hz, Wz = z.shape
        pooled = None
        a_amax = ops.new_amax(z.device) if (not defer and z.is_cuda and ops.split_f16() and ops.split_enabled()
                                            and ops.conv_algo() in ("auto", "split", "bf16")) else None
        act_slots = ops.new_amax(z.device) if (defer and ops.split_f16()) else None
        if want_pool is not None and ops.FUSE_POOL and Hz % 2 == 0 and Wz % 4 == 0:
            pooled = (torch.empty((Bz, C, Hz // 2, Wz // 2), dtype=torch.float32, device=z.device), None)

        def apply(zg, sv, o, sl):
            nonlocal pooled
            if defer:
                return None
            if pooled is not None:
                if o is None:
                    o = torch.empty_like(zg)
                if ops.bn_relu_apply_pool(zg, sv, o, pooled[0][sl], amax=a_amax):
                    return o
                pooled = None
            return ops.bn_relu_apply(zg, sv, out=o, amax=a_amax)

        if G == 1:
            if training:
                ops.bn_train_coeffs(z, gamma, beta, running_mean, running_var, momentum, eps,
                                    cm=None if cm is None else (cm, 0, cm.shape[1]), save=save_all[0], act_slots=act_slots)
            else:
                ops.bn_eval_coeffs(gamma, beta, running_mean, running_var, eps, save=save_all[0])
            a = apply(z, save_all[0], dst, slice(0, Bz))
            if defer:
                a = ops.fp32_placeholder(z.shape, z.device)
        else:
            B = z.shape[0]
            Bg = B // G
            a = dst if dst is not None else (ops.fp32_placeholder(z.shape, z.device) if defer else torch.empty_like(z))
            for g in range(G):
                zg = z[g * Bg:(g + 1) * Bg]
                npg = 0 if cm is None else cm.shape[1] // G
                ops.bn_train_coeffs(zg, gamma, beta, running_mean, running_var, momentum, eps,
                                    cm=None if cm is None else (cm, g * npg, npg), save=save_all[g], act_slots=act_slots)
                apply(zg, save_all[g], None if defer else a[g * Bg:(g + 1) * Bg], slice(g * Bg, (g + 1) * Bg))
        if aux is not None:
            aux["a_amax"] = a_amax
        ctx.twin = ops.twin_src_of(x)
        below = (link_in.pop("z"), link_in.pop("save")) if (training and link_in is not None and "z" in link_in) else (None, None)
        ctx.save_for_backward(x, z, save_all, None if norm is None else norm[0], None if norm is None else norm[1], *below)
        ctx.training = training
        ctx.packed = packed
        ctx.wshape = tuple(weight.shape)
        _record_versions(ctx, weight, gamma, beta)
        ctx.link_out = ctx.link_in = None
        if training and link_out is not None:
            link_out.clear()
            link_out.update(z=z, save=save_all)
            if defer:
                link_out["deferred"] = True
                link_out["slots"] = act_slots
            ctx.link_out = link_out
        if below[0] is not None:
            ctx.link_in = link_in
        if pooled is not None and link_out is not None:
            link_out["pooled"] = pooled
        return a

    @staticmethod
    def _forward_pre(ctx, x, weight, gamma, beta, running_mean, running_var, training, momentum, eps, packed, groups, link_out,
                     link_in, p16, aux=None):
        want_pool = link_out.pop("want_pool", None) if link_out is not None else None
        if link_out is not None:
            link_out.pop("defer", None)
        xP = p16.get("x")
        x_slots = p16.get("x_slots") if xP is not None else None
        if xP is not None:
            z, cm = ops.conv3x3_pre_bn_partials(xP, packed, x_slots)
        else:
            x_amax = aux.get("x_amax") if aux is not None else None
            z, cm = ops.conv3x3_fwd_bn_partials(x, packed, amax=x_amax) if training else (ops.conv3x3_auto(x, packed, 0, amax=x_amax), None)
        G = groups if (training and groups > 1) else 1
        Bz, C, Hz, Wz = z.shape
        Bg = Bz // G
        save_all = torch.empty((G, 4, C), dtype=torch.float32, device=z.device)
        want = bool(p16.get("want"))
        keep = bool(p16.get("keep_fp32")) or not want or ops.PRESPLIT_KEEP_FP32
        aP = None
        if want:
            aP = p16.get("out")
            if aP is None:
                aP = ops.p16_empty(Bz, C, Hz, Wz, z.device)
        head = p16.get("head_link")
        defer_head = bool(head is not None and training and G == 2 and not want and want_pool is None and z.dtype == torch.float32
                          and ops.HEAD_NORM and not ops.PRESPLIT_KEEP_FP32)
        a = torch.empty(z.shape, dtype=torch.float32, device=z.device) if (keep and not defer_head) else ops.fp32_placeholder(z.shape, z.device)
        parts2 = ops.p16_parts() == 2
        act_slots = ops.new_amax(z.device) if (want and parts2 and training) else None
        a_amax = ops.new_amax(z.device) if (not want and parts2) else None
        pooled = None
        if want_pool is not None and Hz % 2 == 0 and Wz % 2 == 0:
            if want_pool.get("p16"):
                pooled = (None, None, ops.p16_empty(Bz, C, Hz // 2, Wz // 2, z.device))
            else:
                pooled = (torch.empty((Bz, C, Hz // 2, Wz // 2), dtype=torch.float32, device=z.device), None, None)
        if training and cm is not None:
            ops.bn_train_coeffs(z[:Bg], gamma, beta, running_mean, running_var, momentum, eps, cm=(cm, 0, cm.shape[1] // G), save=save_all,
                                act_slots=act_slots, groups=G)
        else:
            for g in range(G):
                if training:
                    ops.bn_train_coeffs(z[g * Bg:(g + 1) * Bg], gamma, beta, running_mean, running_var, momentum, eps, save=save_all[g],
                                        act_slots=act_slots)
                else:
                    ops.bn_eval_coeffs(gamma, beta, running_mean, running_var, eps, save=save_all[g])
        gi = Bg if G > 1 else 0
        if defer_head:
            head["z"], head["save"] = z, save_all
            head["bwd_fuse"] = xP is not None
            a_amax = None
        elif pooled is not None:
            if not ops.bn_relu_apply_pool_split(z, save_all, aP, a if keep else None, pooled[2], pooled[0], slots=act_slots, group_images=gi):
                raise RuntimeError("onet_amd: pre-split BatchNorm + pooling pass refused a shape ops.pre_layer_ok accepted")
        elif aP is not None:
            ops.bn_relu_apply_split(z, save_all, aP, a=a if keep else None, slots=act_slots, group_images=gi)
        else:
            ops.bn_relu_apply(z, save_all, out=a, amax=a_amax, group_images=gi)
        p16["a"], p16["a_slots"], p16["a_amax"] = aP, act_slots, a_amax
        ctx.x_slots = x_slots
        ctx.up_link = p16.get("up_link")
        ctx.up_want = None if ctx.up_link is None else ctx.up_link.get("want")
        ctx.twin = ops.twin_src_of(x)
        ctx.head_link = head if defer_head else None
        below = (link_in.pop("z"), link_in.pop("save")) if (training and link_in is not None and "z" in link_in) else (None, None)
        ctx.save_for_backward(x, z, save_all, xP, *below)
        ctx.pre = True
        ctx.training = training
        ctx.packed = packed
        ctx.wshape = tuple(weight.shape)
        _record_versions(ctx, weight, gamma, beta)
        ctx.link_out = ctx.link_in = None
        if training and link_out is not None:
            link_out.clear()
            link_out.update(z=z, save=save_all)
            ctx.link_out = link_out
        if below[0] is not None:
            ctx.link_in = link_in
        if pooled is not None and link_out is not None:
            link_out["pooled"] = pooled
        return a

    @staticmethod
    def _retag_twin(ctx, x):
        tw = getattr(ctx, "twin", None)
        if tw is not None and x is not None and ops.twin_src_of(x) is None:
            x._onet_twin_src = [tw[0], tw[1], None]
        return x

    @staticmethod
    def _take_head_handoff(link, da):
        if link is None or "gl" not in link:
            return None
        rda, rec4, da_amax, gl = link.pop("da"), link.pop("rec4"), link.pop("da_amax", None), link.pop("gl")
        if not ops.is_placeholder(da) or rda.data_ptr() != da.data_ptr() or rda.shape != da.shape or rda.stride() != da.stride():
            raise RuntimeError("onet_amd: the head kept the gradient of the last activation unwritten, but autograd handed its unit "
                               "another tensor (a second consumer of that activation?)")
        return rec4, da_amax, gl

    @staticmethod
    def _backward_pre(ctx, da):
        x, z, save_all, xP, z_below, save_below = ctx.saved_tensors
        x = ConvBNReLUFn._retag_twin(ctx, x)
        need_x, need_w, need_g, need_b = ctx.needs_input_grad[:4]
        _check_versions(ctx, (True, True, False))
        pw, pg, pb = ctx.params
        aff = (ops.grad_slot_if_free(pg) if need_g else None, ops.grad_slot_if_free(pb) if need_b else None)
        rec4, da_amax = None, None
        lk = ctx.link_out
        if lk is not None and "rec4" in lk:
            rda, rec4, da_amax = lk.pop("da"), lk.pop("rec4", None), lk.pop("da_amax", None)
            lk.pop("rec", None)
            if rda.data_ptr() != da.data_ptr() or rda.shape != da.shape or rda.stride() != da.stride():
                rec4 = da_amax = None
        da_gl = None
        hand = ConvBNReLUFn._take_head_handoff(getattr(ctx, "head_link", None), da)
        if hand is not None:
            rec4, da_amax, da_gl = hand
        nones = (None,) * 12
        if xP is None:
            if need_w and not need_x and x.shape[1] <= 4 and ops.STEM_WGRAD_BN and (not ops.is_placeholder(x) or ops.twin_src_of(x) is not None):
                dw, dgamma, dbeta = ops.stem_wgrad_bn(x, da, z, save_all, ctx.training, ctx.wshape, affine_out=aff, rec4=rec4,
                                                      out=ops.grad_slot_if_free(pw))
                return (None, dw, (dgamma if need_g else None), (dbeta if need_b else None)) + nones
            dz, dgamma, dbeta = ops.bn_relu_bwd_groups(da, z, save_all, ctx.training, affine_out=aff, rec4=rec4)
            dw = ops.conv3x3_wgrad_auto(x, dz, ctx.wshape, out=ops.grad_slot_if_free(pw)) if need_w else None
            dx = ops.conv3x3_auto(dz, ctx.packed, 1) if need_x else None
            return (dx, dw, (dgamma if need_g else None), (dbeta if need_b else None)) + nones
        dzP, dz_slots, dgamma, dbeta = ops.bn_relu_bwd_split(da, z, save_all, ctx.training, need_affine_grads=(need_g or need_b),
                                                             affine_out=aff, rec4=rec4, da_amax=da_amax, da_gl=da_gl)
        s1, s2, sc = ops._slots3(getattr(ctx, "x_slots", None))
        dw = ops.conv3x3_split_wgrad_pre(xP, dzP, ctx.wshape, out=ops.grad_slot_if_free(pw), x_slots=s1, dz_slots=dz_slots, x_slots2=s2,
                                         split_ch=sc) if need_w else None
        dpack = ctx.packed.get_pack("split" if dzP.shape[3] == 2 else "plain16")[1]
        dx = None
        if need_x and z_below is not None and save_below is not None and ctx.training:
            fused = ops.conv3x3_split_dgrad_pre_bnreduce(dzP, dpack, ctx.wshape[1], z_below, save_below, slots=dz_slots,
                                                         always=dz_slots is not None, want_amax=ops.p16_parts() == 2)
            if fused is not None:
                dx, rec_below, am_below = fused
                ctx.link_in["da"], ctx.link_in["rec4"] = dx, rec_below
                if am_below is not None:
                    ctx.link_in["da_amax"] = am_below
        up = getattr(ctx, "up_link", None)
        if need_x and dx is None and up is not None and ctx.up_want and (dz_slots is not None or dzP.shape[3] == 1):
            C2, Ct = ctx.up_want
            bound = ops.conv3x3_dgrad_bound(pw, dz_slots, C2) if dzP.shape[3] == 2 else None
            dx, dyP = ops.conv3x3_split_dgrad_pre_slots(dzP, dpack, ctx.wshape[1], C2, bound, slots=dz_slots, always=dz_slots is not None)
            up["dyP"], up["dy_slots"], up["da"] = dyP, bound, dx
        if need_x and dx is None:
            dx = ops.conv3x3_split_pre(dzP, dpack, ctx.wshape[1], slots=dz_slots, always=dz_slots is not None)
        return (dx, dw, (dgamma if need_g else None), (dbeta if need_b else None)) + nones

    @staticmethod
    def backward(ctx, da):
        if ctx.pre:
            return ConvBNReLUFn._backward_pre(ctx, da)
        x, z, save_all, nz, nsave, z_below, save_below = ctx.saved_tensors
        x = ConvBNReLUFn._retag_twin(ctx, x)
        need_x, need_w, need_g, need_b = ctx.needs_input_grad[:4]
        _check_versions(ctx, (True, True, False))
        pw, pg, pb = ctx.params
        aff = (ops.grad_slot_if_free(pg) if need_g else None, ops.grad_slot_if_free(pb) if need_b else None)
        G = save_all.shape[0]
        rec = rec4 = None
        lk = ctx.link_out
        if lk is not None and ("rec" in lk or "rec4" in lk):
            rda, rec, rec4 = lk.pop("da"), lk.pop("rec", None), lk.pop("rec4", None)
            if rda.data_ptr() != da.data_ptr() or rda.shape != da.shape or rda.stride() != da.stride():
                rec = rec4 = None
        Bz, Cz, Hz, Wz = z.shape
        dz_amax = ops.new_amax(z.device) if (ops.grad_f16() and ops.conv_algo() in ("auto", "split", "bf16")
                                             and ops.split_enabled() and Wz >= 16) else None
        if G == 1:
            dz, dgamma, dbeta = ops.bn_relu_bwd(da, z, save_all[0], ctx.training, need_affine_grads=(need_g or need_b),
                                                affine_out=aff, red=None if rec is None else (rec, 0, rec.shape[1]),
                                                red4=None if rec4 is None else (rec4, 0, rec4.shape[0]), amax=dz_amax)
        else:
            Bg = z.shape[0] // G
            dz = torch.empty_like(z)
            dgamma = dbeta = None
            for g in range(G):
                sl = slice(g * Bg, (g + 1) * Bg)
                npg = 0 if rec is None else rec.shape[1] // G
                np4 = 0 if rec4 is None else rec4.shape[0] // G
                _, dgamma, dbeta = ops.bn_relu_bwd(da[sl], z[sl], save_all[g], ctx.training, need_affine_grads=True,
                                                   out=dz[sl], acc=None if g == 0 else (dgamma, dbeta),
                                                   affine_out=aff if g == 0 else None,
                                                   red=None if rec is None else (rec, g * npg, npg),
                                                   red4=None if rec4 is None else (rec4, g * np4, np4), amax=dz_amax)
        if need_w and nz is not None:
            dw = ops.conv3x3_split_wgrad(nz, dz, ctx.wshape, out=ops.grad_slot_if_free(pw), norm=nsave, dz_amax=dz_amax)
        else:
            dw = ops.conv3x3_wgrad_auto(x, dz, ctx.wshape, out=ops.grad_slot_if_free(pw), dz_amax=dz_amax) if need_w else None
        dx = None
        if need_x:
            lk = ctx.link_in
            fused = None
            if lk is not None and z_below is not None:
                fused = ops.conv3x3_dgrad_bnreduce(dz, ctx.packed, z_below, save_below)
            if fused is not None:
                dx, r = fused
# ... 404 lines not shown
```

### onet_amd/ops.py

```python
from __future__ import annotations

import torch

from . import _lib

F32 = torch.float32


import os as _os


def _flags_from_env():
    out = {}
    for item in _os.environ.get("ONET_FLAGS", "").split(","):
        if "=" in item:
            k, v = item.split("=", 1)
            out[k.strip()] = v.strip()
    return out


_FLAGS = _flags_from_env()


def _flag(name, default):
# ... 564 lines not shown
        algo = "auto_nosplit"
    if algo == "auto" and split_enabled() and _split_legal(Cin, Cout, H, W):
        if B * -(-H // 16) * -(-W // 32) * -(-Cout // 64) >= (n_cu() * 3) // 4:
            return "split"
    if algo == "auto_nosplit":
        algo = "auto"
    if algo == "bf16":
        if Cin % 16 == 0 and Cout % 4 == 0 and W >= 16 and H >= 8:
            return "bf16"
        algo = "auto"
    if algo == "direct" or not _wino_legal(Cin, Cout):
        return "direct"
    if min(H, W) < 8:
        return "direct"
    if algo == "winograd4":
        return "winograd4"
    if min(H, W) >= 16:
        img = 1 if W > 16 else 2
        blocks = -(-B // img) * -(-W // (32 if W > 16 else 16)) * -(-H // 16) * -(-Cout // 64)
        if blocks >= (n_cu() * 7) // 8:
            return "winograd4"
    return "direct"


def use_winograd(Cin, Cout, H, W):
    return conv_algo() != "direct" and _wino_legal(Cin, Cout) and min(H, W) >= 8


class Packed3x3(dict):

    def __init__(self, w):
        super().__init__(Cin=w.shape[1], Cout=w.shape[0])
        self.w = w.detach()

    def get_pack(self, algo):
        if algo not in self:
            self[algo] = {"direct": pack3x3, "winograd4": pack3x3_winograd4, "split": pack3x3_split, "plain16": pack3x3_plain16}[algo](self.w)
        return self[algo]


def pack3x3_auto(w):
    return Packed3x3(w)


def _fp32_algo(B, Cin, Cout, H, W):
    algo = conv3x3_algo(B, Cin, Cout, H, W)
    if algo != "bf16":
        return algo
    cur = active_settings()
    with using(cur.replace(conv="auto") if cur is not None else Settings(conv="auto")):
        return conv3x3_algo(B, Cin, Cout, H, W)


def conv3x3_auto(x, pk, direction, out=None, amax=None):
    Ci, Co = (pk["Cin"], pk["Cout"]) if direction == 0 else (pk["Cout"], pk["Cin"])
    shp = x.shape
    algo = _fp32_algo(shp[0], Ci, Co, shp[2], shp[3])
    if algo == "split" and direction == 1 and not split_dgrad():
        with using(active_settings().replace(split=False) if active_settings() is not None else Settings(split=False)):
            algo = _fp32_algo(shp[0], Ci, Co, shp[2], shp[3])
    wq = pk.get_pack(algo)[direction]
    if algo == "winograd4":
        return conv3x3_winograd4(x, wq, Co, out=out)
    if algo == "split":
        if direction == 0 and amax is None and wq.dtype == torch.float16:
            amax = absmax_slots(x)
        return conv3x3_split(x, wq, Co, out=out, amax=amax, always=direction == 1)
    return conv_fwd(x, wq, Co, 3, out=out)


BN_ON_LOAD = _flag("BN_ON_LOAD", True)
BN_ON_LOAD_MAX_COUT = 128
CONVT_SPLIT_MIN_BLOCKS = None
CONVT_SPLIT = _flag("CONVT_SPLIT", True)
SPLIT_F16 = _flag("SPLIT_F16", True)
SPLIT_DGRAD = _flag("SPLIT_DGRAD", True)
PRESPLIT = _flag("PRESPLIT", True)
PRESPLIT_W16 = _flag("PRESPLIT_W16", True)
PRESPLIT_KEEP_FP32 = _flag("PRESPLIT_KEEP_FP32", False)
SPLIT_GRAD_F16 = _flag("SPLIT_GRAD_F16", False)
SPLIT_WGRAD_MINW = 16
SPLIT_AUTO = _flag("SPLIT", True)
STEM_FUSED = _flag("STEM_FUSED", True)


def conv3x3_fwd_bn_partials(x, pk, norm=None, amax=None):
    Ci, Co = pk["Cin"], pk["Cout"]
    if norm is not None:
        z_prev, save, slots = norm
        require_gpu(z_prev, save)
        zs, zbs = plane(z_prev)
        B, _, H, W = zs.shape
        nparts = int(_lib.load().onet_conv3x3_split_nparts(B, H, W)) if not sync_bn() else 0
        out = torch.empty((B, Co, H, W), dtype=F32, device=zs.device)
        cm = torch.empty((Co, nparts, 3), dtype=F32, device=zs.device) if nparts > 0 else None
        e0 = _prof_begin("conv3x3_split_kernel")
        wq = pk.get_pack("split")[0]
        f16 = wq.dtype == torch.float16
        _lib.call("onet_conv3x3_split_fwd_norm", _p(zs), zbs, _p(save), save.shape[0], _p(wq), int(f16), _p(slots) if f16 else None,
                  _p(out), Co * H * W, _p(cm), B, Ci, Co, H, W, _stream())
        _prof_end("conv3x3_split_kernel", 2.0 * B * H * W * Ci * Co * 9, e0, 4.0 * (B * H * W * (Ci + Co) + 9 * Ci * Co))
        return out, cm
    B, _, H, W = x.shape
    if Ci <= 4 and stem_fused() and not sync_bn() and hasattr(pk, "w"):
        nparts = int(_lib.load().onet_conv3x3_stem_nparts(B, Ci, Co, H, W))
        if nparts > 0:
            require_gpu(x)
            tw = twin_src_of(x)
            xs, xbs = plane(tw[0] if tw is not None else x)
            w = pk.w if pk.w.is_contiguous() else pk.w.contiguous()
            out = torch.empty((B, Co, H, W), dtype=F32, device=x.device)
            cm = torch.empty((Co, nparts, 3), dtype=F32, device=x.device)
            e0 = _prof_begin("stem_conv_stats_kernel")
            _lib.call("onet_conv3x3_stem_fwd_stats", _p(xs), xbs, _p(w), _p(out), Co * H * W, _p(cm), B, Ci, Co, H, W,
                      B // 2 if tw is not None else 0, tw[1] if tw is not None else 0.0, _stream())
            _prof_end("stem_conv_stats_kernel", 2.0 * B * H * W * Ci * Co * 9, e0, 4.0 * (B * H * W * (Ci + Co) + 9 * Ci * Co))
            return out, cm
    algo = _fp32_algo(B, Ci, Co, H, W)
    nparts = 0
    if algo == "winograd4" and not sync_bn():
        nparts = int(_lib.load().onet_conv3x3_winograd4_nparts(B, H, W))
    if algo == "split" and not sync_bn():
        nparts = int(_lib.load().onet_conv3x3_split_nparts(B, H, W))
        if nparts > 0:
            wq = pk.get_pack(algo)[0]
            require_gpu(x)
            xs, xbs = plane(x)
            if xs.data_ptr() % 16 or xbs % 4:
                xs = xs.contiguous()
                xbs = xs.stride(0) if B > 1 else xs[0].numel()
            out = torch.empty((B, Co, H, W), dtype=F32, device=x.device)
            cm = torch.empty((Co, nparts, 3), dtype=F32, device=x.device)
            if wq.dtype == torch.float16 and amax is None:
                amax = absmax_slots(xs)
            e0 = _prof_begin("conv3x3_split_kernel")
            if wq.dtype == torch.float16:
                _lib.call("onet_conv3x3_split_conv_amax", _p(xs), xbs, _p(amax), 0, _p(wq), _p(out), Co * H * W, _p(cm), B, Ci, Co, H, W,
                          _stream())
            else:
                _lib.call("onet_conv3x3_split_fwd_stats", _p(xs), xbs, _p(wq), 0, _p(out), Co * H * W, _p(cm), B, Ci, Co, H, W, _stream())
            _prof_end("conv3x3_split_kernel", 2.0 * B * H * W * Ci * Co * 9, e0, 4.0 * (B * H * W * (Ci + Co) + 9 * Ci * Co))
            return out, cm
    if nparts <= 0:
        return conv3x3_auto(x, pk, 0, amax=amax), None
    wq = pk.get_pack(algo)[0]
    require_gpu(x, wq)
    x, xbs = plane(x)
    out = torch.empty((B, Co, H, W), dtype=F32, device=x.device)
    cm = torch.empty((Co, nparts, 3), dtype=F32, device=x.device)
    e0 = _prof_begin("conv_wino4_kernel")
    _lib.call("onet_conv3x3_winograd4_fwd_stats", _p(x), xbs, _p(wq), _p(out), Co * H * W, _p(cm), B, Ci, Co, H, W,
              _stream())
    _prof_end("conv_wino4_kernel", 2.0 * B * H * W * Ci * Co * 9, e0, 4.0 * (B * H * W * (Ci + Co) + 9 * Ci * Co))
    return out, cm


FUSE_BN_REDUCE = _flag("FUSE_BN_REDUCE", True)


def conv3x3_dgrad_bnreduce(dz, pk, z_prev, save_prev):
    if not FUSE_BN_REDUCE or sync_bn():
        return None
    Ci, Co = pk["Cout"], pk["Cin"]
    B, _, H, W = dz.shape
    if conv3x3_algo(B, Ci, Co, H, W) != "winograd4":
        return None
# ... 298 lines not shown
              _p(save), _p(slots), xs.shape[3], group_images, B, C, H, W, _stream(),
              nbytes=(z.element_size() + 2 * xs.shape[3] + 4 * (a is not None)) * z.numel())


def bn_relu_apply_pool_split(z, save, xs, a, ys, y, slots=None, group_images=0):
    z, zbs = plane(z)
    B, C, H, W = z.shape
    assert group_images == 0 or (B % group_images == 0 and save.numel() == (B // group_images) * 4 * C and save.is_contiguous())
    n, m = C * H * W, C * (H // 2) * (W // 2)
    rc = _lib.load().onet_bn_relu_apply_pool_split(_p(z), _z16(z), zbs, _p(xs), 0 if xs is None else _pbs(xs), _p(a),
                                                  0 if a is None else (a.stride(0) if B > 1 else n), _p(ys), 0 if ys is None else _pbs(ys),
                                                  _p(y), 0 if y is None else (y.stride(0) if B > 1 else m), _p(save), _p(slots),
                                                  (xs if xs is not None else ys).shape[3] if (xs is not None or ys is not None) else 2,
                                                  group_images, B, C, H, W, _stream())
    if rc < 0:
        raise _lib.OnetHipError(f"onet_bn_relu_apply_pool_split failed ({rc}): {_lib.last_error()}")
    return rc == 0


def conv3x3_pre_bn_partials(xP, pk, slots=None):
    B, C8, H, np_, W, _ = xP.shape
    Co = pk["Cout"]
    wq = pk.get_pack("split" if np_ == 2 else "plain16")[0]
    nparts = int(_lib.load().onet_conv3x3_split_pre_nparts(B, H, W))
    cm = torch.empty((Co, nparts, 3), dtype=F32, device=xP.device) if nparts > 0 else None
    s1, s2, sc = _slots3(slots)
    return conv3x3_split_pre(xP, wq, Co, slots=s1, stats=cm, slots2=s2, split_ch=sc, z16=cm is not None and np_ == 1 and z16_storage()), cm


def _bn_bwd_groups(da, dabs, z, zbs, save_all, training, affine_out, rec4, da_amax, dz_slots):
    B, C, H, W = z.shape
    HW = H * W
    G = save_all.shape[0]
    Bg = B // G
    dev = z.device
    assert B % G == 0 and save_all.is_contiguous()
    if rec4 is None:
        nparts = _bn_nparts(Bg, HW)
        rec4 = torch.empty((G * nparts, C, 4), dtype=F32, device=dev)
        _lib.call("onet_bn_relu_bwd_reduce", _p(da), dabs, _p(z), _z16(z), zbs, _p(save_all), _p(rec4), G * nparts, _p(da_amax), Bg if G > 1 else 0,
                  B, C, HW, _stream(), nbytes=(4 + z.element_size()) * z.numel())
    else:
        assert rec4.shape[0] % G == 0 and rec4.shape[1] == C and rec4.shape[2] == 4 and rec4.is_contiguous()
    og, ob = affine_out if affine_out is not None else (None, None)
    dgamma = torch.empty(C, dtype=F32, device=dev) if og is None else og
    dbeta = torch.empty(C, dtype=F32, device=dev) if ob is None else ob
    coef = torch.empty((G, 4, C), dtype=F32, device=dev) if training else None
    _lib.call("onet_bn_bwd_finalize", _p(rec4), rec4.shape[0] // G, Bg * HW, _p(dgamma), _p(dbeta), _p(coef), 0, G, C, _p(save_all),
              _p(da_amax), _p(dz_slots), _stream())
    return coef, dgamma, dbeta


def bn_relu_bwd_split(da, z, save_all, training, need_affine_grads=True, affine_out=None, rec=None, rec4=None, da_amax=None, da_gl=None):
    if da_gl is not None:
        if rec4 is None or _z16(z) or (p16_parts() == 2 and da_amax is None):
            raise RuntimeError("onet_amd: a BatchNorm backward on an unmaterialised g * L needs the records of the fused head backward")
        gmap = da_gl[0]
        da, dabs = plane(da_gl[1])
        assert gmap.is_contiguous() and gmap.shape[0] == z.shape[0] and gmap.numel() == z.shape[0] * z.shape[2] * z.shape[3] and da.shape == z.shape
    else:
        da, dabs = plane(da)
    z, zbs = plane(z)
    B, C, H, W = z.shape
    G = save_all.shape[0]
    dev = z.device
    np_ = p16_parts()
    dzP = p16_empty(B, C, H, W, dev, np_)
    scaled = np_ == 2
    dz_slots = new_amax(dev) if scaled else None
    if scaled and rec4 is not None and da_amax is None:
        da_amax = absmax_slots(da)
    if rec4 is None:
        da_amax = new_amax(dev) if scaled else None
    coef, dgamma, dbeta = _bn_bwd_groups(da, dabs, z, zbs, save_all, training, affine_out, rec4, da_amax, dz_slots)
    if da_gl is not None:
        _lib.call("onet_bn_relu_bwd_apply_split_gl", _p(da), dabs, _p(gmap), _p(z), zbs, _p(save_all), _p(coef), _p(dzP), _pbs(dzP), _p(dz_slots), np_,
                  B // G if G > 1 else 0, B, C, H, W, _stream(), nbytes=(8 + 2 * np_) * z.numel() + 4 * gmap.numel())
        return dzP, dz_slots, dgamma, dbeta
    _lib.call("onet_bn_relu_bwd_apply_split", _p(da), dabs, _p(z), _z16(z), zbs, _p(save_all), _p(coef), _p(dzP), _pbs(dzP), _p(dz_slots), np_,
              B // G if G > 1 else 0, B, C, H, W, _stream(), nbytes=(4 + z.element_size() + 2 * np_) * z.numel())
    return dzP, dz_slots, dgamma, dbeta


def stem_wgrad_bn(x, da, z, save_all, training, dw_shape, affine_out=None, rec4=None, out=None, twin=None):
    require_gpu(x, da, z)
    if twin is None:
        twin = twin_src_of(x)
    B, Cin, H, W = x.shape
    x, xbs = plane(twin[0] if twin is not None else x)
    da, dabs = plane(da)
    z, zbs = plane(z)
    Cout = z.shape[1]
    G = save_all.shape[0]
    coef, dgamma, dbeta = _bn_bwd_groups(da, dabs, z, zbs, save_all, training, affine_out, rec4, None, None)
    dw = torch.empty(dw_shape, dtype=F32, device=x.device) if out is None else out
    ws = workspace(_lib.load().onet_conv_wgrad_ws_bytes(B, Cin, Cout, H, W, 3), x.device)
    e0 = _prof_begin("conv_wgrad_kernel")
    _lib.call("onet_conv3x3_stem_wgrad_bn", _p(x), xbs, _p(da), dabs, _p(z), zbs, _p(save_all), _p(coef), B // G if G > 1 else 0, _p(dw),
              _p(ws), ws.numel() * 4, B, Cin, Cout, H, W, 0, B // 2 if twin is not None else 0, twin[1] if twin is not None else 0.0, _stream())
    _prof_end("conv_wgrad_kernel", 2.0 * B * H * W * Cin * Cout * 9, e0, 4.0 * (B * H * W * (Cin + 2 * Cout) + 9 * Cin * Cout))
    return dw, dgamma, dbeta


STEM_WGRAD_BN = _flag("STEM_WGRAD_BN", True)


def bn_relu_bwd_groups(da, z, save_all, training, affine_out=None, rec4=None):
    da, dabs = plane(da)
    z, zbs = plane(z)
    B, C, H, W = z.shape
    G = save_all.shape[0]
    coef, dgamma, dbeta = _bn_bwd_groups(da, dabs, z, zbs, save_all, training, affine_out, rec4, None, None)
    dz = torch.empty((B, C, H, W), dtype=F32, device=z.device)
    _lib.call("onet_bn_relu_bwd_apply", _p(da), dabs, _p(z), zbs, _p(save_all), _p(coef), _p(dz), C * H * W, None, B // G if G > 1 else 0,
              B, C, H * W, _stream(), nbytes=12 * z.numel())
    return dz, dgamma, dbeta


def split_wgrad_ok(x, dz):
    B, Cin, H, W = x.shape
    ok = bool(_lib.load().onet_conv3x3_split_wgrad_ok(B, Cin, dz.shape[1], H, W)) and \
        x.stride(0) % 4 == 0 and x.data_ptr() % 16 == 0 and dz.is_contiguous() and dz.data_ptr() % 16 == 0 and \
        max(Cin, dz.shape[1]) * H * W * 4 < 2 ** 31
    if ok and W < 64:
        ok = ((B - 1) * x.stride(0) + Cin * H * W) * 4 < 2 ** 31 and B * dz.shape[1] * H * W * 4 < 2 ** 31
    return ok


def norm_on_load_ok(B, Cmid, Cout, H, W, groups):
    if not _setting("bn_on_load", BN_ON_LOAD) or sync_bn() or conv_algo() not in ("auto", "split") or groups not in (1, 2) or B % groups:
        return False
    if conv3x3_algo(B, Cmid, Cout, H, W) != "split" or W < SPLIT_WGRAD_MINW:
        return False
    if Cout > BN_ON_LOAD_MAX_COUT:
        return False
    if not _lib.load().onet_conv3x3_split_wgrad_ok(B, Cmid, Cout, H, W) or max(Cmid, Cout) * H * W * 4 >= 2 ** 31:
        return False
    return W >= 64 or B * max(Cmid, Cout) * H * W * 4 < 2 ** 31


def conv3x3_split_wgrad(x, dz, dw_shape, out=None, norm=None, dz_amax=None, x_amax=None):
    if dz_amax is not None:
        require_gpu(x, dz)
        x, xbs = plane(x)
        dz, dzbs = plane(dz)
        B, Cin, H, W = x.shape
        Cout = dz.shape[1]
        dw = torch.empty(dw_shape, dtype=F32, device=x.device) if out is None else out
        ws = workspace(_lib.load().onet_conv3x3_split_wgrad_ws_bytes(B, Cin, Cout, H, W), x.device)
        e0 = _prof_begin("conv3x3_split_wgrad_kernel")
        _lib.call("onet_conv3x3_split_wgrad_f16", _p(x), xbs, _p(x_amax), _p(norm), 0 if norm is None else norm.shape[0], _p(dz), dzbs,
                  _p(dz_amax), _p(dw), _p(ws), ws.numel() * 4, B, Cin, Cout, H, W, 0, _stream())
        _prof_end("conv3x3_split_wgrad_kernel", 2.0 * B * H * W * Cin * Cout * 9, e0, 4.0 * (B * H * W * (Cin + Cout) + 9 * Cin * Cout))
        return dw
    if norm is not None:
        require_gpu(x, dz, norm)
        x, xbs = plane(x)
        dz, dzbs = plane(dz)
        B, Cin, H, W = x.shape
        Cout = dz.shape[1]
        dw = torch.empty(dw_shape, dtype=F32, device=x.device) if out is None else out
        ws = workspace(_lib.load().onet_conv3x3_split_wgrad_ws_bytes(B, Cin, Cout, H, W), x.device)
        e0 = _prof_begin("conv3x3_split_wgrad_kernel")
        _lib.call("onet_conv3x3_split_wgrad_norm", _p(x), xbs, _p(norm), norm.shape[0], _p(dz), dzbs, _p(dw), _p(ws), ws.numel() * 4,
                  B, Cin, Cout, H, W, 0, _stream())
        _prof_end("conv3x3_split_wgrad_kernel", 2.0 * B * H * W * Cin * Cout * 9, e0, 4.0 * (B * H * W * (Cin + Cout) + 9 * Cin * Cout))
        return dw
    require_gpu(x, dz)
    x, xbs = plane(x)
    dz, dzbs = plane(dz)
    B, Cin, H, W = x.shape
    Cout = dz.shape[1]
    dw = torch.empty(dw_shape, dtype=F32, device=x.device) if out is None else out
    need = _lib.load().onet_conv3x3_split_wgrad_ws_bytes(B, Cin, Cout, H, W)
    ws = workspace(need, x.device)
    e0 = _prof_begin("conv3x3_split_wgrad_kernel")
    _lib.call("onet_conv3x3_split_wgrad", _p(x), xbs, _p(dz), dzbs, _p(dw), _p(ws), ws.numel() * 4, B, Cin, Cout, H, W, 0, _stream())
    _prof_end("conv3x3_split_wgrad_kernel", 2.0 * B * H * W * Cin * Cout * 9, e0, 4.0 * (B * H * W * (Cin + Cout) + 9 * Cin * Cout))
    return dw


def _engine_accumulates(param):
    try:
# ... 22 lines not shown
    dw = torch.empty(dw_shape, dtype=F32, device=x.device) if out is None else out
    need = _lib.load().onet_conv3x3_winograd4_wgrad_ws_bytes(B, Cin, Cout, H, W)
    ws = workspace(need, x.device)
    e0 = _prof_begin("conv_wino4_wgrad_kernel")
    _lib.call("onet_conv3x3_winograd4_wgrad", _p(x), xbs, _p(dz), dzbs, _p(dw), _p(ws), ws.numel() * 4, B, Cin, Cout, H, W,
              0, _stream())
    _prof_end("conv_wino4_wgrad_kernel", 2.0 * B * H * W * Cin * Cout * 9, e0, 4.0 * (B * H * W * (Cin + Cout) + 9 * Cin * Cout))
    return dw


def winograd4_wgrad_ok(x, dz):
    B, Cin, H, W = x.shape
    return bool(_lib.load().onet_conv3x3_winograd4_wgrad_ok(B, Cin, dz.shape[1], H, W)) and \
        x.stride(0) % 4 == 0 and x.data_ptr() % 16 == 0 and dz.is_contiguous()


def conv3x3_wgrad_auto(x, dz, dw_shape, out=None, dz_amax=None, x_amax=None):
    Cout, Cin = dw_shape[0], dw_shape[1]
    if conv_algo() in ("auto", "split", "bf16") and (split_enabled() or conv_algo() == "split") and Cin >= 16 and \
            x.shape[3] >= SPLIT_WGRAD_MINW and split_wgrad_ok(x, dz):
        return conv3x3_split_wgrad(x, dz, dw_shape, out=out, dz_amax=dz_amax if grad_f16() else None, x_amax=x_amax)
    if use_winograd(Cin, Cout, x.shape[2], x.shape[3]) and winograd4_wgrad_ok(x, dz):
        return conv3x3_winograd4_wgrad(x, dz, dw_shape, out=out)
    return conv_wgrad(x, dz, dw_shape, 3, out=out)


def conv_fwd(x, wp, Cout, ks, out=None):
    require_gpu(x, wp)
    x, xbs = plane(x)
    B, Cin, H, W = x.shape
    if out is None:
        out = torch.empty((B, Cout, H, W), dtype=F32, device=x.device)
    zbs = out.stride(0) if B > 1 else Cout * H * W
    e0 = _prof_begin("conv_fwd_kernel")
    _lib.call("onet_conv_fwd", _p(x), xbs, _p(wp), _p(out), zbs, None, B, Cin, Cout, H, W, ks, _stream())
    _prof_end("conv_fwd_kernel", 2.0 * B * H * W * Cin * Cout * ks * ks, e0,
              4.0 * (B * H * W * (Cin + Cout) + ks * ks * Cin * Cout))
    return out


def conv_wgrad(x, dz, dw_shape, ks, out_layout=0, out=None):
    require_gpu(x, dz)
    x, xbs = plane(x)
    dz, dzbs = plane(dz)
    B, Cin, H, W = x.shape
    Cout = dz.shape[1]
    dw = torch.empty(dw_shape, dtype=F32, device=x.device) if out is None else out
    need = _lib.load().onet_conv_wgrad_ws_bytes(B, Cin, Cout, H, W, ks)
    ws = workspace(need, x.device)
    e0 = _prof_begin("conv_wgrad_kernel")
    _lib.call("onet_conv_wgrad", _p(x), xbs, _p(dz), dzbs, _p(dw), _p(ws), ws.numel() * 4, B, Cin, Cout, H, W, ks,
              out_layout, 0, _stream())
    _prof_end("conv_wgrad_kernel", 2.0 * B * H * W * Cin * Cout * ks * ks, e0,
              4.0 * (B * H * W * (Cin + Cout) + ks * ks * Cin * Cout))
    return dw


SYNC_BN = False


def set_sync_bn(flag: bool):
    global SYNC_BN
    SYNC_BN = bool(flag)


def _gather_partials(part):
    import torch.distributed as dist
    if not (sync_bn() and dist.is_available() and dist.is_initialized() and dist.get_world_size() > 1):
        return part, 1
    world = dist.get_world_size()
    out = torch.empty((world * part.shape[0],) + tuple(part.shape[1:]), dtype=part.dtype, device=part.device)
    if dist.get_backend() == "nccl":
        dist.all_gather_into_tensor(out, part.contiguous())
    else:
        dist.all_gather(list(out.chunk(world, dim=0)), part.contiguous())
    return out, world


def _bn_nparts(B, HW):
    return B * max(1, (HW + 16383) // 16384)


def bn_train_coeffs(z, gamma, beta, running_mean, running_var, momentum, eps, cm=None, save=None, act_slots=None, groups=1):
    z, zbs = plane(z)
    B, C, H, W = z.shape
    if B * H * W <= 1:
        raise ValueError(f"Expected more than 1 value per channel when training, got input size {list(z.shape)}")
    if cm is not None:
        rec, first, count = cm
        assert rec.shape[0] == C and rec.shape[2] == 3 and 0 <= first and first + count <= rec.shape[1]
        if save is None:
            save = torch.empty((4, C), dtype=F32, device=z.device)
        assert groups == 1 or (first + groups * count <= rec.shape[1] and save.shape[0] == groups and save.is_contiguous())
        _lib.call("onet_bn_finalize_cm", rec.data_ptr() + first * 12, count, rec.shape[1] * 3, _p(gamma), _p(beta),
                  _p(running_mean), _p(running_var), float(momentum), float(eps), _p(save), _p(act_slots), groups, C, _stream())
        return save
    assert groups == 1
    nparts = _bn_nparts(B, H * W)
    part = torch.empty((nparts, C, 3), dtype=F32, device=z.device)
    _lib.call("onet_bn_stats_partial", _p(z), zbs, _p(part), nparts, B, C, H * W, _stream(), nbytes=4 * z.numel())
    part, world = _gather_partials(part)
    nparts *= world
    if save is None:
        save = torch.empty((4, C), dtype=F32, device=z.device)
    _lib.call("onet_bn_finalize", _p(part), nparts, B * H * W * world, _p(gamma), _p(beta), _p(running_mean),
              _p(running_var), float(momentum), float(eps), _p(save), _p(act_slots), C, _stream())
    return save


def bn_eval_coeffs(gamma, beta, running_mean, running_var, eps, save=None):
    C = running_mean.numel()
    if save is None:
        save = torch.empty((4, C), dtype=F32, device=running_mean.device)
    _lib.call("onet_bn_eval_coeffs", _p(gamma), _p(beta), _p(running_mean), _p(running_var), float(eps), _p(save),
              C, _stream())
    return save


def amax_of(t):
    tag = getattr(t, "_onet_amax", None)
    if tag is None:
        return None
    slots, ver = tag
    return slots if ver == t._version else None


def tag_amax(t, slots):
    if slots is not None and t is not None:
        t._onet_amax = (slots, t._version)
    return t


def bn_relu_apply(z, save, out=None, amax=None, group_images=0):
    z, zbs = plane(z)
    B, C, H, W = z.shape
    assert group_images == 0 or (B % group_images == 0 and save.numel() == (B // group_images) * 4 * C and save.is_contiguous())
    if out is None:
        out = torch.empty((B, C, H, W), dtype=F32, device=z.device)
    abs_ = out.stride(0) if B > 1 else C * H * W
    _lib.call("onet_bn_relu_apply", _p(z), _z16(z), zbs, _p(out), abs_, _p(save), _p(amax), group_images,
              B, C, H * W, _stream(), nbytes=(4 + z.element_size()) * z.numel())
    return out


FUSE_POOL = _flag("FUSE_POOL", True)


def bn_relu_apply_pool(z, save, out, y, amax=None):
    z, zbs = plane(z)
    B, C, H, W = z.shape
    if H % 2 or W % 4:
        return False

    def bs(t, n):
        return 0 if t is None else (t.stride(0) if B > 1 else n)
    n, m = C * H * W, C * (H // 2) * (W // 2)
    rc = _lib.load().onet_bn_relu_apply_pool(_p(z), zbs, _p(out), bs(out, n), _p(y), bs(y, m), _p(save), _p(amax), B, C, H, W, _stream())
    if rc < 0:
        raise _lib.OnetHipError(f"onet_bn_relu_apply_pool failed ({rc}): {_lib.last_error()}")
    return rc == 0


def bn_bwd_coefs(da, z, save, training, need_affine_grads=True, acc=None, affine_out=None, red=None, red4=None, da_amax=None):
    da, dabs = plane(da)
    z, zbs = plane(z)
    B, C, H, W = z.shape
    HW = H * W
# ... 378 lines not shown
```

Baseline: 581.7.

## Recompute stem conv pre-activation instead of storing it in forward and backward

```diff
diff --git a/include/onet_hip.h b/include/onet_hip.h
--- a/include/onet_hip.h
+++ b/include/onet_hip.h
@@ -110,6 +110,14 @@
 int onet_conv3x3_stem_nparts(int B, int Cin, int Cout, int H, int W);
 int onet_conv3x3_stem_fwd_stats(const float* x, int64_t x_bs, const float* w, float* z, int64_t z_bs, float* part, int B, int Cin,
                                 int Cout, int H, int W, int twin_B, float twin_bias, void* stream);
+int onet_conv3x3_stem_stats(const float* x, int64_t x_bs, const float* w, float* part, int B, int Cin, int Cout, int H, int W, int twin_B,
+                            float twin_bias, void* stream);
+int onet_conv3x3_stem_bn_relu_split(const float* x, int64_t x_bs, const float* w, void* xs, int64_t xs_bs, const float* save,
+                                    const void* act_amax, int nparts, int group_images, int B, int Cin, int Cout, int H, int W, int twin_B,
+                                    float twin_bias, void* stream);
+int onet_conv3x3_stem_bn_bwd_reduce(const float* x, int64_t x_bs, const float* w, const float* da, int64_t da_bs, const float* save, float* part2,
+                                    int nparts, void* da_amax, int group_images, int B, int Cin, int Cout, int H, int W, int twin_B,
+                                    float twin_bias, void* stream);
 
 int onet_conv3x3_winograd4_wgrad_ok(int B, int Cin, int Cout, int H, int W);
 int64_t onet_conv3x3_winograd4_wgrad_ws_bytes(int B, int Cin, int Cout, int H, int W);
@@ -122,6 +130,9 @@
 int onet_conv3x3_stem_wgrad_bn(const float* x, int64_t x_bs, const float* da, int64_t da_bs, const float* z, int64_t z_bs, const float* save,
                                const float* coef, int group_images, float* dw, void* ws, int64_t ws_bytes, int B, int Cin, int Cout, int H,
                                int W, int accumulate, int twin_B, float twin_bias, void* stream);
+int onet_conv3x3_stem_wgrad_bn_rz(const float* x, int64_t x_bs, const float* da, int64_t da_bs, const float* w, const float* save,
+                                  const float* coef, int group_images, float* dw, void* ws, int64_t ws_bytes, int B, int Cin, int Cout, int H,
+                                  int W, int accumulate, int twin_B, float twin_bias, void* stream);
 int64_t onet_conv_wgrad_ws_bytes(int B, int Cin, int Cout, int H, int W, int ks);
 
 int onet_bn_stats_partial(const float* z, int64_t z_bs, float* part, int nparts,
diff --git a/onet_amd/csrc/bn.hip b/onet_amd/csrc/bn.hip
--- a/onet_amd/csrc/bn.hip
+++ b/onet_amd/csrc/bn.hip
@@ -1,5 +1,5 @@
 #include <type_traits>
-#include "common.hpp"
+#include "stem_tile.hpp"
 
 using namespace onet;
 
@@ -418,6 +418,56 @@
         for (int k = 0; k < 8; ++k) *reinterpret_cast<float4*>(d + (int64_t)k * HW) = make_float4(v[0][k], v[1][k], v[2][k], v[3][k]);
     }
     bn_store_slots_block(tr, xs + (int64_t)b * xs_bs, c8, H, W, blk * 1024, HW, v, s_act, np);
+}
+
+struct StemSplitArgs {
+    const float* x;
+    int64_t x_bs;
+    unsigned* xs;
+    int64_t xs_bs;
+    const unsigned* slots;
+    int B, C, H, W, tilesX, tilesY, np, gimg;
+    int twin_B;
+    float twin_bias;
+};
+
+template <int CIN>
+__global__ __launch_bounds__(256) void stem_conv_bn_relu_split_kernel(StemSplitArgs a, const float* __restrict__ w ,
+                                                                      const float* __restrict__ save_all ) {
+    __shared__ float tile[CIN][ST_LR][ST_LC];
+    float s_inv;
+    const float s_act = a.np == 1 ? 1.f : amax_scale(amax_read(a.slots), false, s_inv);
+    int bid = blockIdx.x;
+    const int tx = bid % a.tilesX;
+    bid /= a.tilesX;
+    const int ty = bid % a.tilesY;
+    const int b = bid / a.tilesY;
+    const int y0 = ty * ST_TH, x0 = tx * ST_TW;
+    const int C = a.C, H = a.H, W = a.W, np = a.np;
+    const float* __restrict__ save = save_all + (a.gimg ? (int64_t)(b / a.gimg) * 4 * C : 0);
+    const bool comp = a.twin_B > 0 && b >= a.twin_B;
+    const float* xb = a.x + (int64_t)(comp ? b - a.twin_B : b) * a.x_bs;
+    bn_u32x4* const tr = bn_tr_lds();
+    float win[CIN][3][6];
+    stem_load_window<CIN>(tile, xb, H, W, y0, x0, comp, a.twin_bias, win);
+    unsigned* xsb = a.xs + (int64_t)b * a.xs_bs;
+#pragma unroll 1
+    for (int c8 = 0; c8 < (C >> 3); ++c8) {
+        float v[4][8];
+#pragma unroll
+        for (int k = 0; k < 8; ++k) {
+            const int c = c8 * 8 + k;
+            const float mean = save[c], sc = save[2 * C + c], sh = save[3 * C + c];
+            float acc[4];
+            stem_z4<CIN>(w + (int64_t)c * CIN * 9, win, acc);
+#pragma unroll
+            for (int j = 0; j < 4; ++j) v[j][k] = fmaxf(fmaf(acc[j] - mean, sc, sh), 0.f);
+        }
+        if (c8) __syncthreads();
+        bn_store_slots_block_fn(tr, xsb, np == 2 ? W : 0, v, s_act, [&](int px) -> int64_t {
+            return ((int64_t)(c8 * H + y0 + (px >> 6)) * np) * W + x0 + (px & 63);
+        }, np);
+    }
 }
 
 template <typename ZT = float>
@@ -639,6 +689,98 @@
         o[1] = (float)(v[0] - (double)o[0]);
         o[2] = (float)v[1];
         o[3] = (float)(v[1] - (double)o[2]);
+    }
+}
+
+struct StemReduceArgs {
+    const float* x;
+    int64_t x_bs;
+    const float* w;
+    const float* da;
+    int64_t da_bs;
+    const float* save;
+    float* part2;
+    unsigned* amax;
+    int C, H, W, chunks, chunk_len, gimg;
+    int twin_B;
+    float twin_bias;
+};
+
+template <int CIN, int CG>
+__global__ __launch_bounds__(256) void stem_bn_bwd_reduce_kernel(StemReduceArgs a) {
+    __shared__ double red[8 * CG];
+    const int C = a.C, H = a.H, W = a.W, HW = H * W;
+    const int cgs = (C + CG - 1) / CG;
+    const int c0 = (blockIdx.x % cgs) * CG, p = blockIdx.x / cgs;
+    const int b = p / a.chunks, ch = p % a.chunks;
+    const float* save = a.save + (a.gimg ? (int64_t)(b / a.gimg) * 4 * C : 0);
+    const bool comp = a.twin_B > 0 && b >= a.twin_B;
+    const float* xb = a.x + (int64_t)(comp ? b - a.twin_B : b) * a.x_bs;
+    const float* ds = a.da + (int64_t)b * a.da_bs;
+    const bool xvec = (a.x_bs & 3) == 0 && (reinterpret_cast<uintptr_t>(a.x) & 15) == 0;
+    const int beg = ch * a.chunk_len, end = min(beg + a.chunk_len, HW);
+    float vmax = 0.f;
+    double v[2 * CG];
+#pragma unroll
+    for (int g = 0; g < 2 * CG; ++g) v[g] = 0.0;
+    for (int i = beg + threadIdx.x * 4; i < end; i += 1024) {
+        const int y = i / W, x = i - y * W;
+        float win[CIN][3][6];
+#pragma unroll
+        for (int ci = 0; ci < CIN; ++ci)
+#pragma unroll
+            for (int dy = 0; dy < 3; ++dy) {
+                const int yy = y - 1 + dy;
+                const bool rowok = yy >= 0 && yy < H;
+                const float* r = xb + (int64_t)ci * HW + (int64_t)(rowok ? yy : 0) * W;
+                float (&o)[6] = win[ci][dy];
+                if (xvec) {
+                    const float4 m = *reinterpret_cast<const float4*>(r + x);
+                    o[1] = m.x; o[2] = m.y; o[3] = m.z; o[4] = m.w;
+                } else {
+#pragma unroll
+                    for (int k = 0; k < 4; ++k) o[1 + k] = r[x + k];
+                }
+                o[0] = x > 0 ? r[x - 1] : 0.f;
+                o[5] = x + 4 < W ? r[x + 4] : 0.f;
+#pragma unroll
+                for (int k = 0; k < 6; ++k) {
+                    const bool ok = rowok && x - 1 + k >= 0 && x - 1 + k < W;
+                    float t = o[k];
+                    if (comp) t = fminf(fmaxf(1.f - t + a.twin_bias, 0.f), 1.f);
+                    o[k] = ok ? t : 0.f;
+                }
+            }
+#pragma unroll
+        for (int g = 0; g < CG; ++g) {
+            const int c = min(c0 + g, C - 1);
+            const float mean = save[c], invstd = save[C + c], sc = save[2 * C + c], sh = save[3 * C + c];
+            const double meand = mean, invd = invstd;
+            const float4 gq = *reinterpret_cast<const float4*>(ds + (int64_t)c * HW + i);
+            const float gg[4] = {gq.x, gq.y, gq.z, gq.w};
+            float zz[4];
+            stem_z4<CIN>(a.w + (int64_t)c * CIN * 9, win, zz);
+#pragma unroll
+            for (int e = 0; e < 4; ++e) {
+                const double dy = fmaf(zz[e] - mean, sc, sh) > 0.f ? (double)gg[e] : 0.0;
+                v[2 * g] += dy;
+                v[2 * g + 1] += dy * (((double)zz[e] - meand) * invd);
+                if (c0 + g < C) vmax = fmaxf(vmax, fabsf(gg[e]));
+            }
+        }
+    }
+    amax_commit(vmax, a.amax);
+    block_sum_256<double, 2 * CG>(v, red);
+    if (threadIdx.x == 0) {
+#pragma unroll
+        for (int g = 0; g < CG; ++g) {
+            if (c0 + g >= C) break;
+            float* o = a.part2 + ((int64_t)p * C + c0 + g) * 4;
+            o[0] = (float)v[2 * g];
+            o[1] = (float)(v[2 * g] - (double)o[0]);
+            o[2] = (float)v[2 * g + 1];
+            o[3] = (float)(v[2 * g + 1] - (double)o[2]);
+        }
     }
 }
 
@@ -953,6 +1095,57 @@
     return check_launch("bn_relu_bwd_reduce_kernel");
 }
 
+int onet_conv3x3_stem_bn_relu_split(const float* x, int64_t x_bs, const float* w, void* xs, int64_t xs_bs, const float* save,
+                                    const void* act_amax, int nparts, int group_images, int B, int Cin, int Cout, int H, int W, int twin_B,
+                                    float twin_bias, void* stream) {
+    ONET_REQUIRE(nparts == 1 || nparts == 2, "conv3x3_stem_bn_relu_split: nparts must be 2 (fp16 hi | mid) or 1 (plain bf16)");
+    ONET_REQUIRE(x && w && xs && save && group_images >= 0, "conv3x3_stem_bn_relu_split: bad args");
+    ONET_REQUIRE(stem_nparts(B, Cin, Cout, H, W) > 0 && (Cout % 8) == 0,
+                 "conv3x3_stem_bn_relu_split: needs 1 <= Cin <= 4, Cout %% 8 == 0, Cout <= %d and a map made of full 16 x 64 tiles", ST_MAXC);
+    ONET_REQUIRE(x_bs >= (int64_t)Cin * H * W, "conv3x3_stem_bn_relu_split: batch stride too small");
+    ONET_REQUIRE((reinterpret_cast<uintptr_t>(xs) & 15) == 0 && (xs_bs & 3) == 0, "conv3x3_stem_bn_relu_split: 16-byte aligned slots required");
+    ONET_REQUIRE(xs_bs >= (int64_t)Cout * H * W * nparts / 2, "conv3x3_stem_bn_relu_split: slot batch stride too small");
+    ONET_REQUIRE(group_images == 0 || B % group_images == 0, "conv3x3_stem_bn_relu_split: B must be a multiple of group_images");
+    ONET_REQUIRE(twin_B == 0 || 2 * twin_B == B, "conv3x3_stem_bn_relu_split: a twin batch holds twin_B = B / 2 images in memory");
+    StemSplitArgs a{x, x_bs, (unsigned*)xs, xs_bs, (const unsigned*)act_amax, B, Cout, H, W, W / ST_TW, H / ST_TH, nparts, group_images,
+                    twin_B, twin_bias};
+    const dim3 g((unsigned)((int64_t)B * a.tilesX * a.tilesY)), t(256);
+    const unsigned lds = bn_tr_bytes(nparts);
+    switch (Cin) {
+        case 1: hipLaunchKernelGGL(stem_conv_bn_relu_split_kernel<1>, g, t, lds, as_stream(stream), a, w, save); break;
+        case 2: hipLaunchKernelGGL(stem_conv_bn_relu_split_kernel<2>, g, t, lds, as_stream(stream), a, w, save); break;
+        case 3: hipLaunchKernelGGL(stem_conv_bn_relu_split_kernel<3>, g, t, lds, as_stream(stream), a, w, save); break;
+        default: hipLaunchKernelGGL(stem_conv_bn_relu_split_kernel<4>, g, t, lds, as_stream(stream), a, w, save); break;
+    }
+    return check_launch("stem_conv_bn_relu_split_kernel");
+}
+
+int onet_conv3x3_stem_bn_bwd_reduce(const float* x, int64_t x_bs, const float* w, const float* da, int64_t da_bs, const float* save, float* part2,
+                                    int nparts, void* da_amax, int group_images, int B, int Cin, int Cout, int H, int W, int twin_B,
+                                    float twin_bias, void* stream) {
+    ONET_REQUIRE(x && w && da && save && part2 && B > 0 && Cin >= 1 && Cin <= 4 && Cout > 0 && H > 0 && W > 0 && group_images >= 0,
+                 "conv3x3_stem_bn_bwd_reduce: bad args (1 <= Cin <= 4)");
+    ONET_REQUIRE((int64_t)H * W < (1 << 30) && (W & 3) == 0 && (da_bs & 3) == 0 && (reinterpret_cast<uintptr_t>(da) & 15) == 0,
+                 "conv3x3_stem_bn_bwd_reduce: W %% 4 == 0 and 16-byte aligned gradient rows required");
+    ONET_REQUIRE(x_bs >= (int64_t)Cin * H * W && da_bs >= (int64_t)Cout * H * W, "conv3x3_stem_bn_bwd_reduce: batch stride too small");
+    ONET_REQUIRE(group_images == 0 || B % group_images == 0, "conv3x3_stem_bn_bwd_reduce: B must be a multiple of group_images");
+    ONET_REQUIRE(twin_B == 0 || 2 * twin_B == B, "conv3x3_stem_bn_bwd_reduce: a twin batch holds twin_B = B / 2 images in memory");
+    int chunks, chunk_len;
+    ONET_REQUIRE(split_plan(nparts, B, H * W, chunks, chunk_len), "conv3x3_stem_bn_bwd_reduce: nparts=%d must be a multiple of B=%d", nparts, B);
+    StemReduceArgs a{x, x_bs, w, da, da_bs, save, part2, (unsigned*)da_amax, Cout, H, W, chunks, chunk_len, group_images, twin_B, twin_bias};
+    constexpr int CG = 8;
+    const int64_t blocks = (int64_t)nparts * cdiv(Cout, CG);
+    ONET_REQUIRE(blocks < (1ll << 31), "conv3x3_stem_bn_bwd_reduce: grid too large");
+    const dim3 g((unsigned)blocks), t(256);
+    switch (Cin) {
+        case 1: hipLaunchKernelGGL((stem_bn_bwd_reduce_kernel<1, CG>), g, t, 0, as_stream(stream), a); break;
+        case 2: hipLaunchKernelGGL((stem_bn_bwd_reduce_kernel<2, CG>), g, t, 0, as_stream(stream), a); break;
+        case 3: hipLaunchKernelGGL((stem_bn_bwd_reduce_kernel<3, CG>), g, t, 0, as_stream(stream), a); break;
+        default: hipLaunchKernelGGL((stem_bn_bwd_reduce_kernel<4, CG>), g, t, 0, as_stream(stream), a); break;
+    }
+    return check_launch("stem_bn_bwd_reduce_kernel");
+}
+
 int onet_bn_bwd_bound(const float* save, const float* coef, const void* da_amax, int64_t count, void* dz_amax, int C, void* stream) {
     ONET_REQUIRE(save && da_amax && dz_amax && count > 0 && C > 0, "bn_bwd_bound: bad args");
     hipLaunchKernelGGL(bn_bwd_bound_kernel, dim3(cdiv(C, 64)), dim3(64), 0, as_stream(stream), save, coef, (const unsigned*)da_amax,
diff --git a/onet_amd/csrc/common.hpp b/onet_amd/csrc/common.hpp
--- a/onet_amd/csrc/common.hpp
+++ b/onet_amd/csrc/common.hpp
@@ -95,6 +95,22 @@
     return __builtin_bit_cast(float, (unsigned)(127 + k) << 23);
 }
 
+template <int CIN>
+__device__ __forceinline__ void stem_z4(const float* __restrict__ w, const float (&win)[CIN][3][6], float (&acc)[4]) {
+#pragma unroll
+    for (int j = 0; j < 4; ++j) acc[j] = 0.f;
+#pragma unroll
+    for (int ci = 0; ci < CIN; ++ci)
+#pragma unroll
+        for (int dy = 0; dy < 3; ++dy)
+#pragma unroll
+            for (int dx = 0; dx < 3; ++dx) {
+                const float wv = w[(ci * 3 + dy) * 3 + dx];
+#pragma unroll
+                for (int j = 0; j < 4; ++j) acc[j] = fmaf(wv, win[ci][dy][dx + j], acc[j]);
+            }
+}
+
 int launch_wgrad_reduce(const float* slab, float* dw, int splitK, int taps, int Cout, int Cin, int out_layout, int accumulate,
                         hipStream_t st);
 
diff --git a/onet_amd/csrc/conv_mfma.hip b/onet_amd/csrc/conv_mfma.hip
--- a/onet_amd/csrc/conv_mfma.hip
+++ b/onet_amd/csrc/conv_mfma.hip
@@ -351,6 +351,7 @@
     const float* bn_save = nullptr;
     const float* bn_coef = nullptr;
     int bn_gimg = 0;
+    const float* bn_w = nullptr;
     int twin_B = 0;
     float twin_bias = 0.f;
 };
@@ -552,7 +553,7 @@
 }
 
 constexpr int STEM_ROWS = 32;
-template <int CIN, int COG, bool BN = false>
+template <int CIN, int COG, bool BN = false, bool RZ = false>
 __global__ __launch_bounds__(256) void conv3x3_stem_wgrad_kernel(WgArgs a) {
     constexpr int NV = COG * CIN * 9;
     __shared__ float red[4][NV];
@@ -565,10 +566,10 @@
     const bool comp = a.twin_B > 0 && b >= a.twin_B;
     const float* xb = a.x + (int64_t)(comp ? b - a.twin_B : b) * a.x_bs;
     const float* dzb = a.dz + (int64_t)b * a.dz_bs + (int64_t)cg * COG * HW;
-    const float* zb = BN ? a.bn_z + (int64_t)b * a.bn_z_bs + (int64_t)cg * COG * HW : nullptr;
+    const float* zb = (BN && !RZ) ? a.bn_z + (int64_t)b * a.bn_z_bs + (int64_t)cg * COG * HW : nullptr;
     const int y0 = yb + wid * (STEM_ROWS / 4), y1 = min(y0 + STEM_ROWS / 4, H);
     const bool vec = (W & 3) == 0 && (a.dz_bs & 3) == 0 && (reinterpret_cast<uintptr_t>(a.dz) & 15) == 0 &&
-                     (!BN || ((a.bn_z_bs & 3) == 0 && (reinterpret_cast<uintptr_t>(a.bn_z) & 15) == 0));
+                     (!BN || RZ || ((a.bn_z_bs & 3) == 0 && (reinterpret_cast<uintptr_t>(a.bn_z) & 15) == 0));
     float bmean[COG], binv[COG], bsc[COG], bsh[COG];
     double bc1[COG], bc2[COG];
     if (BN) {
@@ -630,7 +631,7 @@
                     if (vec) {
                         const float4 q = *reinterpret_cast<const float4*>(dzb + o);
                         gz[0] = q.x; gz[1] = q.y; gz[2] = q.z; gz[3] = q.w;
-                        if (BN) {
+                        if (BN && !RZ) {
                             const float4 r = *reinterpret_cast<const float4*>(zb + o);
                             zz[0] = r.x; zz[1] = r.y; zz[2] = r.z; zz[3] = r.w;
                         }
@@ -639,9 +640,10 @@
                         for (int p = 0; p < 4; ++p)
                             if (x0 + p < W) {
                                 gz[p] = dzb[o + p];
-                                if (BN) zz[p] = zb[o + p];
+                                if (BN && !RZ) zz[p] = zb[o + p];
                             }
                     }
+                    if (RZ) stem_z4<CIN>(a.bn_w + (int64_t)(cg * COG + g) * CIN * 9, win, zz);
                     if (BN) {
 #pragma unroll
                         for (int p = 0; p < 4; ++p) {
@@ -859,6 +861,37 @@
     return check_launch("wgrad_reduce_kernel");
 }
 
+int onet_conv3x3_stem_wgrad_bn_rz(const float* x, int64_t x_bs, const float* da, int64_t da_bs, const float* w, const float* save,
+                                  const float* coef, int group_images, float* dw, void* ws, int64_t ws_bytes, int B, int Cin, int Cout, int H,
+                                  int W, int accumulate, int twin_B, float twin_bias, void* stream) {
+    ONET_REQUIRE(x && da && w && save && dw && ws, "conv3x3_stem_wgrad_bn_rz: null pointer");
+    ONET_REQUIRE(B > 0 && Cin > 0 && Cin <= 4 && Cout > 0 && H > 0 && W > 0 && group_images >= 0 && (group_images == 0 || B % group_images == 0),
+                 "conv3x3_stem_wgrad_bn_rz: bad shape (Cin <= 4)");
+    WgArgs a{x, x_bs, da, da_bs, (float*)ws, B, Cin, Cout, H, W, 1, cdiv(Cout, 64), 1, 1, 1};
+    a.bn_w = w;
+    a.bn_save = save;
+    a.bn_coef = coef;
+    a.bn_gimg = group_images;
+    ONET_REQUIRE(twin_B == 0 || 2 * twin_B == B, "conv3x3_stem_wgrad_bn_rz: a twin batch holds twin_B = B / 2 images in memory");
+    a.twin_B = twin_B;
+    a.twin_bias = twin_bias;
+    const int nb = stem_blocks(B, H);
+    const int64_t need = (int64_t)nb * 9 * Cout * Cin * 4;
+    ONET_REQUIRE(ws_bytes >= need, "conv3x3_stem_wgrad_bn_rz: workspace %lld < %lld bytes", (long long)ws_bytes, (long long)need);
+    hipStream_t st = as_stream(stream);
+    switch (Cin) {
+        case 1: hipLaunchKernelGGL((conv3x3_stem_wgrad_kernel<1, 4, true, true>), dim3(nb * cdiv(Cout, 4)), dim3(256), 0, st, a); break;
+        case 2: hipLaunchKernelGGL((conv3x3_stem_wgrad_kernel<2, 2, true, true>), dim3(nb * cdiv(Cout, 2)), dim3(256), 0, st, a); break;
+        case 3: hipLaunchKernelGGL((conv3x3_stem_wgrad_kernel<3, 2, true, true>), dim3(nb * cdiv(Cout, 2)), dim3(256), 0, st, a); break;
+        default: hipLaunchKernelGGL((conv3x3_stem_wgrad_kernel<4, 1, true, true>), dim3(nb * cdiv(Cout, 1)), dim3(256), 0, st, a); break;
+    }
+    int rc = check_launch("conv3x3_stem_wgrad_kernel");
+    if (rc) return rc;
+    const int64_t n = (int64_t)Cout * Cin;
+    hipLaunchKernelGGL(wgrad_reduce_kernel, dim3((unsigned)cdiv(n, 64), 9u), dim3(256), 0, st, (const float*)ws, dw, nb, 9, Cout, Cin, 0, accumulate);
+    return check_launch("wgrad_reduce_kernel");
+}
+
 int onet_conv_wgrad(const float* x, int64_t x_bs, const float* dz, int64_t dz_bs, float* dw, void* ws,
                     int64_t ws_bytes, int B, int Cin, int Cout, int H, int W, int ks, int out_layout,
                     int accumulate, void* stream) {
diff --git a/onet_amd/csrc/stem.hip b/onet_amd/csrc/stem.hip
--- a/onet_amd/csrc/stem.hip
+++ b/onet_amd/csrc/stem.hip
@@ -1,5 +1,5 @@
 #include <algorithm>
-#include "common.hpp"
+#include "stem_tile.hpp"
 
 using namespace onet;
 
@@ -17,9 +17,6 @@
     float twin_bias;
 };
 
-constexpr int ST_TH = 16, ST_TW = 64, ST_LR = ST_TH + 2, ST_LC = ST_TW + 4;
-constexpr int ST_MAXC = 128;
-
 #define ONET_ST_DPP_ADD(v, ctrl, rmask) \
     v += __builtin_bit_cast(float, __builtin_amdgcn_update_dpp(0, __builtin_bit_cast(int, v), ctrl, rmask, 0xf, false))
 __device__ __forceinline__ float wave_sum_hi(float v) {
@@ -33,7 +30,7 @@
 }
 #undef ONET_ST_DPP_ADD
 
-template <int CIN>
+template <int CIN, bool STORE = true>
 __global__ __launch_bounds__(256) void stem_conv_stats_kernel(StemArgs a) {
     __shared__ float tile[CIN][ST_LR][ST_LC];
     __shared__ float sc[4][ST_MAXC][2];
@@ -47,41 +44,16 @@
     const int HW = a.H * a.W;
     const bool comp = a.twin_B > 0 && b >= a.twin_B;
     const float* xb = a.x + (int64_t)(comp ? b - a.twin_B : b) * a.x_bs;
-
-    for (int i = tid; i < CIN * ST_LR * 66; i += 256) {
-        const int ci = i / (ST_LR * 66), r = (i / 66) % ST_LR, c = i % 66;
-        const int yy = y0 - 1 + r, xx = x0 - 1 + c;
-        const bool ok = yy >= 0 && yy < a.H && xx >= 0 && xx < a.W;
-        float v = ok ? xb[(int64_t)ci * HW + (int64_t)yy * a.W + xx] : 0.f;
-        if (comp && ok) v = fminf(fmaxf(1.f - v + a.twin_bias, 0.f), 1.f);
-        tile[ci][r][c] = v;
-    }
-    __syncthreads();
-
     const int r = tid >> 4, q = tid & 15;
     float win[CIN][3][6];
-#pragma unroll
-    for (int ci = 0; ci < CIN; ++ci)
-#pragma unroll
-        for (int dy = 0; dy < 3; ++dy)
-#pragma unroll
-            for (int dx = 0; dx < 6; ++dx) win[ci][dy][dx] = tile[ci][r + dy][4 * q + dx];
+    stem_load_window<CIN>(tile, xb, a.H, a.W, y0, x0, comp, a.twin_bias, win);
 
-    float* zb = a.z + (int64_t)b * a.z_bs + (int64_t)(y0 + r) * a.W + x0 + 4 * q;
+    float* zb = STORE ? a.z + (int64_t)b * a.z_bs + (int64_t)(y0 + r) * a.W + x0 + 4 * q : nullptr;
     for (int co = 0; co < a.Cout; ++co) {
         const float* wp = a.w + (int64_t)co * CIN * 9;
-        float acc[4] = {0.f, 0.f, 0.f, 0.f};
-#pragma unroll
-        for (int ci = 0; ci < CIN; ++ci)
-#pragma unroll
-            for (int dy = 0; dy < 3; ++dy)
-#pragma unroll
-                for (int dx = 0; dx < 3; ++dx) {
-                    const float wv = wp[(ci * 3 + dy) * 3 + dx];
-#pragma unroll
-                    for (int j = 0; j < 4; ++j) acc[j] = fmaf(wv, win[ci][dy][dx + j], acc[j]);
-                }
-        *reinterpret_cast<float4*>(zb + (int64_t)co * HW) = make_float4(acc[0], acc[1], acc[2], acc[3]);
+        float acc[4];
+        stem_z4<CIN>(wp, win, acc);
+        if (STORE) *reinterpret_cast<float4*>(zb + (int64_t)co * HW) = make_float4(acc[0], acc[1], acc[2], acc[3]);
         if (a.part) {
             const float pv = __builtin_bit_cast(float, __builtin_amdgcn_readfirstlane(__builtin_bit_cast(int, acc[0])));
             float s1 = 0.f, s2 = 0.f;
@@ -122,12 +94,6 @@
     }
 }
 
-int stem_nparts(int B, int Cin, int Cout, int H, int W) {
-    if (B <= 0 || Cin < 1 || Cin > 4 || Cout < 1 || Cout > ST_MAXC || H <= 0 || W <= 0 || (H % ST_TH) || (W % ST_TW)) return 0;
-    const int64_t n = (int64_t)B * (H / ST_TH) * (W / ST_TW);
-    return n < (1 << 30) ? (int)n : 0;
-}
-
 }
 
 extern "C" {
@@ -155,4 +121,24 @@
     return check_launch("stem_conv_stats_kernel");
 }
 
+int onet_conv3x3_stem_stats(const float* x, int64_t x_bs, const float* w, float* part, int B, int Cin, int Cout, int H, int W, int twin_B,
+                            float twin_bias, void* stream) {
+    ONET_REQUIRE(x && w && part, "conv3x3_stem_stats: null pointer");
+    ONET_REQUIRE(stem_nparts(B, Cin, Cout, H, W) > 0,
+                 "conv3x3_stem_stats: needs 1 <= Cin <= 4, Cout <= %d and a map made of full 16 x 64 tiles (onet_conv3x3_stem_nparts() == 0 elsewhere)",
+                 ST_MAXC);
+    ONET_REQUIRE(x_bs >= (int64_t)Cin * H * W, "conv3x3_stem_stats: batch stride too small");
+    ONET_REQUIRE(twin_B == 0 || 2 * twin_B == B, "conv3x3_stem_stats: a twin batch holds twin_B = B / 2 images in memory");
+    StemArgs a{x, x_bs, w, nullptr, 0, part, B, Cout, H, W, W / ST_TW, H / ST_TH, twin_B, twin_bias};
+    const int64_t blocks = (int64_t)B * a.tilesX * a.tilesY;
+    const dim3 g((unsigned)blocks), t(256);
+    switch (Cin) {
+        case 1: hipLaunchKernelGGL((stem_conv_stats_kernel<1, false>), g, t, 0, as_stream(stream), a); break;
+        case 2: hipLaunchKernelGGL((stem_conv_stats_kernel<2, false>), g, t, 0, as_stream(stream), a); break;
+        case 3: hipLaunchKernelGGL((stem_conv_stats_kernel<3, false>), g, t, 0, as_stream(stream), a); break;
+        default: hipLaunchKernelGGL((stem_conv_stats_kernel<4, false>), g, t, 0, as_stream(stream), a); break;
+    }
+    return check_launch("stem_conv_stats_kernel");
 }
+
+}
diff --git a/onet_amd/csrc/stem_tile.hpp b/onet_amd/csrc/stem_tile.hpp
--- /dev/null
+++ b/onet_amd/csrc/stem_tile.hpp
@@ -0,0 +1,37 @@
+#pragma once
+#include "common.hpp"
+
+namespace onet {
+
+constexpr int ST_TH = 16, ST_TW = 64, ST_LR = ST_TH + 2, ST_LC = ST_TW + 4;
+constexpr int ST_MAXC = 128;
+
+template <int CIN>
+__device__ __forceinline__ void stem_load_window(float (&tile)[CIN][ST_LR][ST_LC], const float* __restrict__ xb, int H, int W, int y0, int x0,
+                                                 bool comp, float twin_bias, float (&win)[CIN][3][6]) {
+    const int tid = threadIdx.x, HW = H * W;
+    for (int i = tid; i < CIN * ST_LR * 66; i += 256) {
+        const int ci = i / (ST_LR * 66), r = (i / 66) % ST_LR, c = i % 66;
+        const int yy = y0 - 1 + r, xx = x0 - 1 + c;
+        const bool ok = yy >= 0 && yy < H && xx >= 0 && xx < W;
+        float v = ok ? xb[(int64_t)ci * HW + (int64_t)yy * W + xx] : 0.f;
+        if (comp && ok) v = fminf(fmaxf(1.f - v + twin_bias, 0.f), 1.f);
+        tile[ci][r][c] = v;
+    }
+    __syncthreads();
+    const int r = tid >> 4, q = tid & 15;
+#pragma unroll
+    for (int ci = 0; ci < CIN; ++ci)
+#pragma unroll
+        for (int dy = 0; dy < 3; ++dy)
+#pragma unroll
+            for (int dx = 0; dx < 6; ++dx) win[ci][dy][dx] = tile[ci][r + dy][4 * q + dx];
+}
+
+inline int stem_nparts(int B, int Cin, int Cout, int H, int W) {
+    if (B <= 0 || Cin < 1 || Cin > 4 || Cout < 1 || Cout > ST_MAXC || H <= 0 || W <= 0 || (H % ST_TH) || (W % ST_TW)) return 0;
+    const int64_t n = (int64_t)B * (H / ST_TH) * (W / ST_TW);
+    return n < (1 << 30) ? (int)n : 0;
+}
+
+}
diff --git a/onet_amd/functional.py b/onet_amd/functional.py
--- a/onet_amd/functional.py
+++ b/onet_amd/functional.py
@@ -133,7 +133,13 @@
             link_out.pop("defer", None)
         xP = p16.get("x")
         x_slots = p16.get("x_slots") if xP is not None else None
-        if xP is not None:
+        stem_fwd = bool(xP is None and training and running_mean is not None and running_var is not None and want_pool is None
+                        and p16.get("want") and not p16.get("keep_fp32") and not ops.PRESPLIT_KEEP_FP32 and p16.get("head_link") is None
+                        and ops.stem_recompute_ok(x, packed))
+        stem_rz = bool(stem_fwd and ops.STEM_RECOMPUTE_BWD and not ctx.needs_input_grad[0])
+        if stem_rz:
+            z, cm = ops.fp32_placeholder((x.shape[0], weight.shape[0], x.shape[2], x.shape[3]), x.device), ops.stem_stats(x, packed.w)
+        elif xP is not None:
             z, cm = ops.conv3x3_pre_bn_partials(xP, packed, x_slots)
         else:
             x_amax = aux.get("x_amax") if aux is not None else None
@@ -180,6 +186,8 @@
         elif pooled is not None:
             if not ops.bn_relu_apply_pool_split(z, save_all, aP, a if keep else None, pooled[2], pooled[0], slots=act_slots, group_images=gi):
                 raise RuntimeError("onet_amd: pre-split BatchNorm + pooling pass refused a shape ops.pre_layer_ok accepted")
+        elif stem_fwd:
+            ops.stem_bn_relu_split(x, packed.w, save_all, aP, slots=act_slots, group_images=gi)
         elif aP is not None:
             ops.bn_relu_apply_split(z, save_all, aP, a=a if keep else None, slots=act_slots, group_images=gi)
         else:
@@ -191,7 +199,8 @@
         ctx.twin = ops.twin_src_of(x)
         ctx.head_link = head if defer_head else None
         below = (link_in.pop("z"), link_in.pop("save")) if (training and link_in is not None and "z" in link_in) else (None, None)
-        ctx.save_for_backward(x, z, save_all, xP, *below)
+        ctx.stem_rz = stem_rz
+        ctx.save_for_backward(x, z, save_all, xP, *below, ctx.twin[0] if (stem_rz and ctx.twin is not None) else None)
         ctx.pre = True
         ctx.training = training
         ctx.packed = packed
@@ -200,8 +209,9 @@
         ctx.link_out = ctx.link_in = None
         if training and link_out is not None:
             link_out.clear()
-            link_out.update(z=z, save=save_all)
-            ctx.link_out = link_out
+            if not stem_rz:
+                link_out.update(z=z, save=save_all)
+                ctx.link_out = link_out
         if below[0] is not None:
             ctx.link_in = link_in
         if pooled is not None and link_out is not None:
@@ -227,7 +237,7 @@
 
     @staticmethod
     def _backward_pre(ctx, da):
-        x, z, save_all, xP, z_below, save_below = ctx.saved_tensors
+        x, z, save_all, xP, z_below, save_below, _ = ctx.saved_tensors
         x = ConvBNReLUFn._retag_twin(ctx, x)
         need_x, need_w, need_g, need_b = ctx.needs_input_grad[:4]
         _check_versions(ctx, (True, True, False))
@@ -245,6 +255,13 @@
         if hand is not None:
             rec4, da_amax, da_gl = hand
         nones = (None,) * 12
+        if getattr(ctx, "stem_rz", False):
+            if need_x or not ops.is_placeholder(z):
+                raise RuntimeError("onet_amd: the stem's pre-activation was not stored (ops.STEM_RECOMPUTE_BWD), but this backward needs the "
+                                   "tensor itself (an input gradient of the stem?)")
+            dw, dgamma, dbeta = ops.stem_wgrad_bn(x, da, None, save_all, ctx.training, ctx.wshape, affine_out=aff, rec4=None,
+                                                  out=ops.grad_slot_if_free(pw) if need_w else None, w=pw.detach())
+            return (None, (dw if need_w else None), (dgamma if need_g else None), (dbeta if need_b else None)) + nones
         if xP is None:
             if need_w and not need_x and x.shape[1] <= 4 and ops.STEM_WGRAD_BN and (not ops.is_placeholder(x) or ops.twin_src_of(x) is not None):
                 dw, dgamma, dbeta = ops.stem_wgrad_bn(x, da, z, save_all, ctx.training, ctx.wshape, affine_out=aff, rec4=rec4,
diff --git a/onet_amd/ops.py b/onet_amd/ops.py
--- a/onet_amd/ops.py
+++ b/onet_amd/ops.py
@@ -670,6 +670,65 @@
 SPLIT_WGRAD_MINW = 16
 SPLIT_AUTO = _flag("SPLIT", True)
 STEM_FUSED = _flag("STEM_FUSED", True)
+STEM_RECOMPUTE = _flag("STEM_RECOMPUTE", True)
+STEM_RECOMPUTE_BWD = _flag("STEM_RECOMPUTE_BWD", False)
+
+
+def _stem_operands(x, w, twin=None):
+    tw = twin if twin is not None else twin_src_of(x)
+    xs, xbs = plane(tw[0] if tw is not None else x)
+    return xs, xbs, (w if w.is_contiguous() else w.contiguous()), (x.shape[0] // 2 if tw is not None else 0), (tw[1] if tw is not None else 0.0)
+
+
+def stem_recompute_ok(x, pk):
+    Ci, Co = pk["Cin"], pk["Cout"]
+    B, _, H, W = x.shape
+    if not STEM_RECOMPUTE or not STEM_WGRAD_BN or Ci > 4 or Co % 8 or not stem_fused() or sync_bn() or not hasattr(pk, "w") or not x.is_cuda:
+        return False
+    if is_placeholder(x) and twin_src_of(x) is None:
+        return False
+    return int(_lib.load().onet_conv3x3_stem_nparts(B, Ci, Co, H, W)) > 0
+
+
+def stem_stats(x, w):
+    require_gpu(x, w)
+    B, Ci, H, W = x.shape
+    Co = w.shape[0]
+    xs, xbs, w, tB, tbias = _stem_operands(x, w)
+    nparts = int(_lib.load().onet_conv3x3_stem_nparts(B, Ci, Co, H, W))
+    if nparts <= 0:
+        raise RuntimeError("onet_amd: stem_stats needs a map made of full 16 x 64 tiles (ops.stem_recompute_ok)")
+    cm = torch.empty((Co, nparts, 3), dtype=F32, device=xs.device)
+    e0 = _prof_begin("stem_conv_stats_kernel")
+    _lib.call("onet_conv3x3_stem_stats", _p(xs), xbs, _p(w), _p(cm), B, Ci, Co, H, W, tB, tbias, _stream())
+    _prof_end("stem_conv_stats_kernel", 2.0 * B * H * W * Ci * Co * 9, e0, 4.0 * (B * H * W * Ci + 9 * Ci * Co))
+    return cm
+
+
+def stem_bn_relu_split(x, w, save, xs, slots=None, group_images=0):
+    require_gpu(x, w)
+    B, Ci, H, W = x.shape
+    Co = w.shape[0]
+    assert group_images == 0 or (B % group_images == 0 and save.numel() == (B // group_images) * 4 * Co and save.is_contiguous())
+    xp, xbs, w, tB, tbias = _stem_operands(x, w)
+    _lib.call("onet_conv3x3_stem_bn_relu_split", _p(xp), xbs, _p(w), _p(xs), _pbs(xs), _p(save), _p(slots), xs.shape[3], group_images,
+              B, Ci, Co, H, W, tB, tbias, _stream(), nbytes=(4 * Ci + 2 * xs.shape[3] * Co) * B * H * W)
+
+
+def stem_bn_bwd_reduce(x, w, da, save_all, da_amax=None, twin=None):
+    require_gpu(x, w, da)
+    B, Ci, H, W = x.shape
+    Co = w.shape[0]
+    G = save_all.shape[0]
+    Bg = B // G
+    assert B % G == 0 and save_all.is_contiguous()
+    xp, xbs, w, tB, tbias = _stem_operands(x, w, twin)
+    da, dabs = plane(da)
+    nparts = _bn_nparts(Bg, H * W)
+    rec4 = torch.empty((G * nparts, Co, 4), dtype=F32, device=da.device)
+    _lib.call("onet_conv3x3_stem_bn_bwd_reduce", _p(xp), xbs, _p(w), _p(da), dabs, _p(save_all), _p(rec4), G * nparts, _p(da_amax),
+              Bg if G > 1 else 0, B, Ci, Co, H, W, tB, tbias, _stream(), nbytes=4 * (Ci + Co) * B * H * W)
+    return rec4
 
 
 def conv3x3_fwd_bn_partials(x, pk, norm=None, amax=None):
@@ -1134,8 +1193,10 @@
     return dzP, dz_slots, dgamma, dbeta
 
 
-def stem_wgrad_bn(x, da, z, save_all, training, dw_shape, affine_out=None, rec4=None, out=None, twin=None):
+def stem_wgrad_bn(x, da, z, save_all, training, dw_shape, affine_out=None, rec4=None, out=None, twin=None, w=None):
     require_gpu(x, da, z)
+    if z is None:
+        return _stem_wgrad_bn_rz(x, da, w, save_all, training, dw_shape, affine_out, rec4, out, twin)
     if twin is None:
         twin = twin_src_of(x)
     B, Cin, H, W = x.shape
@@ -1151,6 +1212,34 @@
     _lib.call("onet_conv3x3_stem_wgrad_bn", _p(x), xbs, _p(da), dabs, _p(z), zbs, _p(save_all), _p(coef), B // G if G > 1 else 0, _p(dw),
               _p(ws), ws.numel() * 4, B, Cin, Cout, H, W, 0, B // 2 if twin is not None else 0, twin[1] if twin is not None else 0.0, _stream())
     _prof_end("conv_wgrad_kernel", 2.0 * B * H * W * Cin * Cout * 9, e0, 4.0 * (B * H * W * (Cin + 2 * Cout) + 9 * Cin * Cout))
+    return dw, dgamma, dbeta
+
+
+def _stem_wgrad_bn_rz(x, da, w, save_all, training, dw_shape, affine_out, rec4, out, twin):
+    if w is None:
+        raise RuntimeError("onet_amd: the stem's weight gradient without its pre-activation needs the layer's weight to recompute it")
+    B, Cin, H, W = x.shape
+    Cout = w.shape[0]
+    G = save_all.shape[0]
+    dev = da.device
+    if rec4 is None:
+        rec4 = stem_bn_bwd_reduce(x, w, da, save_all, twin=twin)
+    else:
+        assert rec4.shape[0] % G == 0 and rec4.shape[1] == Cout and rec4.shape[2] == 4 and rec4.is_contiguous()
+    xp, xbs, w, tB, tbias = _stem_operands(x, w, twin)
+    da, dabs = plane(da)
+    og, ob = affine_out if affine_out is not None else (None, None)
+    dgamma = torch.empty(Cout, dtype=F32, device=dev) if og is None else og
+    dbeta = torch.empty(Cout, dtype=F32, device=dev) if ob is None else ob
+    coef = torch.empty((G, 4, Cout), dtype=F32, device=dev) if training else None
+    _lib.call("onet_bn_bwd_finalize", _p(rec4), rec4.shape[0] // G, (B // G) * H * W, _p(dgamma), _p(dbeta), _p(coef), 0, G, Cout, _p(save_all),
+              None, None, _stream())
+    dw = torch.empty(dw_shape, dtype=F32, device=dev) if out is None else out
+    ws = workspace(_lib.load().onet_conv_wgrad_ws_bytes(B, Cin, Cout, H, W, 3), dev)
+    e0 = _prof_begin("conv_wgrad_kernel")
+    _lib.call("onet_conv3x3_stem_wgrad_bn_rz", _p(xp), xbs, _p(da), dabs, _p(w), _p(save_all), _p(coef), B // G if G > 1 else 0, _p(dw),
+              _p(ws), ws.numel() * 4, B, Cin, Cout, H, W, 0, tB, tbias, _stream())
+    _prof_end("conv_wgrad_kernel", 2.0 * B * H * W * Cin * Cout * 9, e0, 4.0 * (B * H * W * (Cin + Cout) + 9 * Cin * Cout))
     return dw, dgamma, dbeta
 
 
@@ -1339,7 +1428,8 @@
 
 
 def bn_train_coeffs(z, gamma, beta, running_mean, running_var, momentum, eps, cm=None, save=None, act_slots=None, groups=1):
-    z, zbs = plane(z)
+    if cm is None:
+        z, zbs = plane(z)
     B, C, H, W = z.shape
     if B * H * W <= 1:
         raise ValueError(f"Expected more than 1 value per channel when training, got input size {list(z.shape)}")
```

After: 583.4, median of 6. Within noise of the previous version (+0.3%).
